# Totoro97/f2-nerf

Measured on AMD Instinct MI355X. Metric: training ray-samples/s (ngp_fox), higher is better.
Workload: dtype f16; 1 GPU; ngp_fox wanjinyou.yaml, 8192 rays/batch/GPU, 2^19 x16 table, the first 2188 iterations of training from the fresh-initialised table (fineness 8.7), synthetic random-pose rays, full train step (fwd+bwd+Adam+octree update); rays_per_batch=8192, parallelism=ray-dp1

## Files before the change

f2-nerf_amd/capi.py:

```python
import ctypes
import os

import torch

from . import build

_lib = None
ABI_VERSION = 13


class F2nError(RuntimeError):
    pass


def lib():
    global _lib
    if _lib is None:
        if not os.path.exists(build.LIB):
            raise F2nError("native library %s is missing: run `python -c 'import __graft_entry__ as g; g.build()'` "
                           "(there is no CPU fallback)" % build.LIB)
        _lib = ctypes.CDLL(build.LIB)
        _lib.f2n_build_info.restype = ctypes.c_char_p
        if _lib.f2n_abi_version() != ABI_VERSION:
            raise F2nError("%s reports ABI version %d, this binding is written for %d: rebuild (__graft_entry__.build())"
# ... 534 lines not shown

def flex_acc_bwd(n_rays, include_this, dsum, se, out):
    _ck(lib().f2n_flex_acc_bwd(_stream(), _i(n_rays), _i(int(include_this)), _p(dsum, "f32"), _p(se, "i32"), _p(out, "f32")),
        "f2n_flex_acc_bwd")


def adam_coefficients(step, lr, beta1=0.9, beta2=0.99, eps=1e-15, weight_decay=0.0, grad_scale=1.0):
    out = (ctypes.c_float * 9)()
    _ck(lib().f2n_adam_coefficients(_i(step), _f(lr), _d(beta1), _d(beta2), _f(eps), _f(weight_decay), _f(grad_scale), out),
        "f2n_adam_coefficients")
    return [float(v) for v in out]


def adam_step(n, param, grad, grad_scale, grad_round_h16, exp_avg, exp_avg_sq, step, lr, beta1, beta2, eps, wd, param_h,
              skip_flag=None, zero_grad=False):
    _ck(lib().f2n_adam_step(_stream(), _i(n), _p(param, "f32"), _p(grad, "f32"), _f(grad_scale), _i(int(grad_round_h16)),
                            _p(exp_avg, "f32"), _p(exp_avg_sq, "f32"), _i(step), _f(lr), _d(beta1), _d(beta2), _f(eps),
                            _f(wd), _p(param_h, "h16", True), _i(int(zero_grad)), _p(skip_flag, "i32", True)), "f2n_adam_step")


class _AdamGroup(ctypes.Structure):
    _fields_ = [("param", ctypes.c_void_p), ("grad", ctypes.c_void_p), ("exp_avg", ctypes.c_void_p), ("exp_avg_sq", ctypes.c_void_p),
                ("param_h", ctypes.c_void_p), ("n", ctypes.c_int), ("grad_scale", ctypes.c_float), ("weight_decay", ctypes.c_float),
                ("grad_round_h16", ctypes.c_int), ("check_finite", ctypes.c_int)]


def adam_small_groups(groups, step, lr, beta1, beta2, eps, zero_grad, flags=None, skip_flag=None):
    arr = (_AdamGroup * len(groups))()
    for a, g in zip(arr, groups):
        a.param = _p(g["param"], "f32").value
        a.grad = _p(g["grad"], "f32").value
        a.exp_avg = _p(g["exp_avg"], "f32").value
        a.exp_avg_sq = _p(g["exp_avg_sq"], "f32").value
        a.param_h = _p(g.get("param_h"), "h16", True).value
        a.n = int(g["param"].numel())
        a.grad_scale = float(g["grad_scale"])
        a.weight_decay = float(g["weight_decay"])
        a.grad_round_h16 = int(bool(g.get("grad_round_h16", False)))
        a.check_finite = int(bool(g.get("check_finite", False)))
    _ck(lib().f2n_adam_small_groups(_stream(), _i(len(groups)), arr, _i(step), _f(lr), _d(beta1), _d(beta2), _f(eps),
                                    _i(int(zero_grad)), _p(flags, "i32", True), _p(skip_flag, "i32", True)), "f2n_adam_small_groups")


def adam_fused(groups, table, step, lr, beta1, beta2, eps, zero_grad, skip_flag=None):
    arr = (_AdamGroup * max(len(groups), 1))()
    for a, g in zip(arr, groups):
        a.param = _p(g["param"], "f32").value
        a.grad = _p(g["grad"], "f32").value
        a.exp_avg = _p(g["exp_avg"], "f32").value
        a.exp_avg_sq = _p(g["exp_avg_sq"], "f32").value
        a.param_h = _p(g.get("param_h"), "h16", True).value
        a.n = int(g["param"].numel())
        a.grad_scale = float(g["grad_scale"])
        a.weight_decay = float(g["weight_decay"])
        a.grad_round_h16 = int(bool(g.get("grad_round_h16", False)))
        a.check_finite = 0
    t = table or {}
    _ck(lib().f2n_adam_fused(_stream(), _i(len(groups)), arr, _i(int(t.get("n", 0))), _p(t.get("param"), "f32", True),
                             _p(t.get("grad_h"), "h16", True), _f(float(t.get("grad_scale", 1.0))), _p(t.get("exp_avg"), "f32", True),
                             _p(t.get("exp_avg_sq"), "f32", True), _p(t.get("param_h"), "h16", True), _i(step), _f(lr), _d(beta1),
                             _d(beta2), _f(eps), _i(int(zero_grad)), _p(skip_flag, "i32", True)), "f2n_adam_fused")


def field_bwd_dyn(n_max, n_dev, n_off, n_volumes, prim_pool, local_idx, local_size, bias_pool, level_scale, pts_warped, volume_idx,
                  vol_stride, mlp_params_h, saved_x_h, dfeat, loss_scale, dparams_scaled, grad_table_h, level_entries, defer_reduce):
    _ck(lib().f2n_field_bwd_dyn(_stream(), _i(n_max), _p(n_dev, "i32", True), _i(n_off), _i(n_volumes), _p(prim_pool, "i32"),
                                _p(local_idx, "i32"), _p(local_size, "i32"), _p(bias_pool, "f32"), _p(level_scale, "f32"),
                                _p(pts_warped, "f32"), _p(volume_idx, "i32"), _i(vol_stride), _p(mlp_params_h, "h16"),
                                _p(saved_x_h, "h16"), _p(dfeat, "f32"), _f(loss_scale), _p(dparams_scaled, "f32"),
                                _p(grad_table_h, "h16"), _i(level_entries), _i(int(defer_reduce))), "f2n_field_bwd_dyn")


def field_bwd_dyn_rows(n_max, n_dev, n_off, n_volumes, prim_pool, local_idx, local_size, bias_pool, level_scale, pts_warped, volume_idx,
                       vol_stride, mlp_params_h, x_edge_h, x_cache_h, src_rows, dfeat, loss_scale, dparams_scaled, grad_table_h,
                       level_entries, defer_reduce):
    _ck(lib().f2n_field_bwd_dyn_rows(_stream(), _i(n_max), _p(n_dev, "i32", True), _i(n_off), _i(n_volumes), _p(prim_pool, "i32"),
                                     _p(local_idx, "i32"), _p(local_size, "i32"), _p(bias_pool, "f32"), _p(level_scale, "f32"),
                                     _p(pts_warped, "f32"), _p(volume_idx, "i32"), _i(vol_stride), _p(mlp_params_h, "h16"),
                                     _p(x_edge_h, "h16", True), _p(x_cache_h, "h16"), _p(src_rows, "i32"), _p(dfeat, "f32"),
                                     _f(loss_scale), _p(dparams_scaled, "f32"), _p(grad_table_h, "h16"), _i(level_entries),
                                     _i(int(defer_reduce))), "f2n_field_bwd_dyn_rows")


class _StepTail(ctypes.Structure):
    _fields_ = [("n_flags_a", ctypes.c_int), ("flags_grad_a", ctypes.c_void_p), ("n_flags_b", ctypes.c_int), ("flags_grad_b", ctypes.c_void_p),
                ("flags", ctypes.c_void_p), ("flags_mirror", ctypes.c_void_p), ("n_groups", ctypes.c_int), ("groups", ctypes.c_void_p),
                ("n_table", ctypes.c_int), ("table_param", ctypes.c_void_p), ("table_exp_avg", ctypes.c_void_p),
                ("table_exp_avg_sq", ctypes.c_void_p), ("table_param_h", ctypes.c_void_p), ("table_grad_scale", ctypes.c_float),
                ("step", ctypes.c_int), ("lr", ctypes.c_float), ("beta1", ctypes.c_double), ("beta2", ctypes.c_double), ("eps", ctypes.c_float),
                ("after_reduce", ctypes.c_void_p), ("after_reduce_user", ctypes.c_void_p), ("leave_table_to_caller", ctypes.c_int)]


def field_bwd_step_tail(n_max, n_dev, n_off, n_volumes, prim_pool, local_idx, local_size, bias_pool, level_scale, pts_warped, volume_idx,
                        vol_stride, mlp_params_h, saved_x_h, dfeat, loss_scale, dparams_scaled, grad_table_h, level_entries, flags_a,
                        flags_b, flags, groups, table, step, lr, beta1, beta2, eps, tail_stream=None, flags_mirror=None, leave_table_to_caller=False,
                        after_reduce=None, x_cache_h=None, src_rows=None):
    arr = (_AdamGroup * max(len(groups), 1))()
    for a, g in zip(arr, groups):
        a.param = _p(g["param"], "f32").value
        a.grad = _p(g["grad"], "f32").value
        a.exp_avg = _p(g["exp_avg"], "f32").value
        a.exp_avg_sq = _p(g["exp_avg_sq"], "f32").value
        a.param_h = _p(g.get("param_h"), "h16", True).value
        a.n = int(g["param"].numel())
        a.grad_scale = float(g["grad_scale"])
        a.weight_decay = float(g["weight_decay"])
        a.grad_round_h16 = int(bool(g.get("grad_round_h16", False)))
        a.check_finite = 0
    t = _StepTail()
    t.n_flags_a, t.flags_grad_a = int(flags_a.numel()), _p(flags_a, "f32").value
    t.n_flags_b, t.flags_grad_b = int(flags_b.numel()), _p(flags_b, "f32").value
    t.flags, t.flags_mirror = _p(flags, "i32").value, _mapped(flags_mirror).value
    t.n_groups, t.groups = len(groups), ctypes.cast(arr, ctypes.c_void_p).value
    t.n_table = int(table["n"])
    t.table_param, t.table_exp_avg, t.table_exp_avg_sq = _p(table["param"], "f32").value, _p(table["exp_avg"], "f32").value, _p(table["exp_avg_sq"], "f32").value
    t.table_param_h, t.table_grad_scale = _p(table["param_h"], "h16").value, float(table["grad_scale"])
    t.step, t.lr, t.beta1, t.beta2, t.eps = int(step), float(lr), float(beta1), float(beta2), float(eps)
    t.leave_table_to_caller = int(bool(leave_table_to_caller))
    cb = None
    if after_reduce is not None:
        cb = ctypes.CFUNCTYPE(None, ctypes.c_void_p, ctypes.c_void_p)(lambda user, chain: after_reduce(chain))
        t.after_reduce = ctypes.cast(cb, ctypes.c_void_p).value
    by_owners = ctypes.c_int(0)
    ts = ctypes.c_void_p(tail_stream.cuda_stream) if tail_stream is not None else ctypes.c_void_p(0)
    if x_cache_h is not None:
        _ck(lib().f2n_field_bwd_step_tail_rows(_stream(), ts, _i(n_max), _p(n_dev, "i32", True), _i(n_off), _i(n_volumes), _p(prim_pool, "i32"),
                                               _p(local_idx, "i32"), _p(local_size, "i32"), _p(bias_pool, "f32"), _p(level_scale, "f32"),
                                               _p(pts_warped, "f32"), _p(volume_idx, "i32"), _i(vol_stride), _p(mlp_params_h, "h16"),
                                               _p(saved_x_h, "h16", True), _p(x_cache_h, "h16"), _p(src_rows, "i32"), _p(dfeat, "f32"),
                                               _f(loss_scale), _p(dparams_scaled, "f32"), _p(grad_table_h, "h16"), _i(level_entries),
                                               ctypes.byref(t), ctypes.byref(by_owners)), "f2n_field_bwd_step_tail_rows")
        return by_owners.value
    _ck(lib().f2n_field_bwd_step_tail(_stream(), ts, _i(n_max), _p(n_dev, "i32", True), _i(n_off), _i(n_volumes), _p(prim_pool, "i32"),
                                      _p(local_idx, "i32"), _p(local_size, "i32"), _p(bias_pool, "f32"), _p(level_scale, "f32"),
                                      _p(pts_warped, "f32"), _p(volume_idx, "i32"), _i(vol_stride), _p(mlp_params_h, "h16"),
                                      _p(saved_x_h, "h16"), _p(dfeat, "f32"), _f(loss_scale), _p(dparams_scaled, "f32"),
                                      _p(grad_table_h, "h16"), _i(level_entries), ctypes.byref(t), ctypes.byref(by_owners)),
        "f2n_field_bwd_step_tail")
    return by_owners.value


def reduce_deferred():
    _ck(lib().f2n_reduce_deferred(_stream()), "f2n_reduce_deferred")


def deferred_reset():
    _ck(lib().f2n_deferred_reset(), "f2n_deferred_reset")


def adam_step_h16grad(n, param, grad_h, grad_scale, exp_avg, exp_avg_sq, step, lr, beta1, beta2, eps, wd, param_h,
                      zero_grad, skip_flag=None):
    _ck(lib().f2n_adam_step_h16grad(_stream(), _i(n), _p(param, "f32"), _p(grad_h, "h16"), _f(grad_scale),
                                    _p(exp_avg, "f32"), _p(exp_avg_sq, "f32"), _i(step), _f(lr), _d(beta1), _d(beta2),
                                    _f(eps), _f(wd), _p(param_h, "h16"), _i(int(zero_grad)),
                                    _p(skip_flag, "i32", True)), "f2n_adam_step_h16grad")


def train_loss(n_rays, pred, gt, disparity, sampled_var, n_edge, feat_dim, edge_feats, var_w, disp_w, tv_w, out_losses,
               dcolors, ddisparity, dvar, dedge_feats):
    _ck(lib().f2n_train_loss(_stream(), _i(n_rays), _p(pred, "f32"), _p(gt, "f32"), _p(disparity, "f32", True),
                             _p(sampled_var, "f32", True), _i(n_edge), _i(feat_dim), _p(edge_feats, "f32", True), _f(var_w),
                             _f(disp_w), _f(tv_w), _p(out_losses, "f32"), _p(dcolors, "f32", True), _p(ddisparity, "f32", True),
                             _p(dvar, "f32", True), _p(dedge_feats, "f32", True)), "f2n_train_loss")


def composite_train(n_rays, se, f0, f0_stride, dt, t, rgb, bg, gt, var_w, disp_w, tv_w, gs_progress, n_edge, feat_dim, edge_feats,
                    dedge_feats, colors, weights, drgb, df0, df0_stride, out_losses, defer_reduce=False):
    _ck(lib().f2n_composite_train(_stream(), _i(n_rays), _p(se, "i32"), _p(f0, "f32"), _i(f0_stride), _p(dt, "f32"), _p(t, "f32"),
                                  _p(rgb, "f32"), _p(bg, "f32"), _p(gt, "f32"), _f(var_w), _f(disp_w), _f(tv_w), _f(gs_progress),
                                  _i(n_edge), _i(feat_dim), _p(edge_feats, "f32", True), _p(dedge_feats, "f32", True),
                                  _p(colors, "f32"), _p(weights, "f32"), _p(drgb, "f32"), _p(df0, "f32"), _i(df0_stride),
                                  _p(out_losses, "f32"), _i(1 if defer_reduce else 0)), "f2n_composite_train")


def nonfinite_flags(n_a, a, n_b, b, flags, mirror=None):
    _ck(lib().f2n_nonfinite_flags_ex(_stream(), _i(n_a), _p(a, "f32", True), _i(n_b), _p(b, "f32", True), _p(flags, "i32"),
                                     _mapped(mirror)), "f2n_nonfinite_flags_ex")


def _lo3(lo):
    return (_f * 3)(*(float(v) for v in lo))


def oct_locate_warp(n, pts_world, tree_nodes, transes, out_pts, out_anchors):
    _ck(lib().f2n_oct_locate_warp(_stream(), _i(n), _p(pts_world, "f32"), _p(tree_nodes, "u8"), _p(transes, "u8"), _p(out_pts, "f32"),
                                  _p(out_anchors, "i32")), "f2n_oct_locate_warp")


def oct_locate_warp_grid(lo, step, nx, ny, nz, first_z, n_z, tree_nodes, transes, out_pts, out_anchors):
    _ck(lib().f2n_oct_locate_warp_grid(_stream(), _lo3(lo), _f(step), _i(nx), _i(ny), _i(nz), _i(first_z), _i(n_z), _p(tree_nodes, "u8"),
                                       _p(transes, "u8"), _p(out_pts, "f32"), _p(out_anchors, "i32")), "f2n_oct_locate_warp_grid")


def located_compact(n, anchors, pts_warped, counts, start_end, total, out_pts, out_vol, out_src=None):
    _ck(lib().f2n_located_compact(_stream(), _i(n), _p(anchors, "i32"), _p(pts_warped, "f32"), _p(counts, "i32"), _p(start_end, "i32"),
                                  _p(total, "i32"), _p(out_pts, "f32"), _p(out_vol, "i32"), _p(out_src, "i32", True)),
        "f2n_located_compact")


def density_scatter(n, anchors, start_end, f0, density):
    _ck(lib().f2n_density_scatter(_stream(), _i(n), _p(anchors, "i32"), _p(start_end, "i32"), _p(f0, "f32"), _p(density, "f32")),
        "f2n_density_scatter")


def field_density_grad(n, n_volumes, table_h, prim_pool, local_idx, local_size, bias_pool, level_scale, pts_warped, volume_idx, vol_stride,
                       mlp_params_h, x_h, out_dx, out_df0_dw):
    _ck(lib().f2n_field_density_grad(_stream(), _i(n), _i(n_volumes), _p(table_h, "h16"), _p(prim_pool, "i32"), _p(local_idx, "i32"),
# ... 550 lines not shown
```

f2-nerf_amd/csrc/field.hip:

```cpp
#include <math.h>
#include <atomic>
#include <string.h>

#include "adam_dev.h"
#include "mlp_dev.h"

struct F2nHashArgs {
  const half_t* table;
  const int32_t* prim_pool;
  const float* bias_pool;
  int n_volumes;
};

struct F2nLevelTab {
  float scale[F2N_N_LEVELS];
  int32_t base[F2N_N_LEVELS];
  uint32_t size[F2N_N_LEVELS];
};

__device__ __forceinline__ void f2n_level_tab_fill(F2nLevelTab& s, const float* level_scale, const int32_t* local_idx,
                                                   const int32_t* local_size, int tid) {
  if (tid < F2N_N_LEVELS) {
    s.scale[tid] = level_scale[tid];
    s.base[tid] = local_idx[tid];
// ... 959 lines not shown
  return f2n_rowfrag(x, F2N_D_IN, s, 0, g);
}
__device__ __forceinline__ half8_t f2n_load_xfrag_f32(const float* __restrict__ x, int s, int g, bool valid) {
  half8_t r = {0, 0, 0, 0, 0, 0, 0, 0};
  if (valid) {
    const float4_t lo = *(const float4_t*) (x + (size_t) s * F2N_D_IN + 4 * g);
    const float4_t hi = *(const float4_t*) (x + (size_t) s * F2N_D_IN + 16 + 4 * g);
#pragma unroll
    for (int i = 0; i < 4; i++) {
      r[i] = (half_t) lo[i];
      r[4 + i] = (half_t) hi[i];
    }
  }
  return r;
}
__device__ __forceinline__ void f2n_store_xfrag_h(half_t* __restrict__ x, int s, int g, half8_t xf) {
  half_t* p = x + (size_t) s * F2N_D_IN + 4 * g;
  *(half4_t*) p = __builtin_shufflevector(xf, xf, 0, 1, 2, 3);
  *(half4_t*) (p + 16) = __builtin_shufflevector(xf, xf, 4, 5, 6, 7);
}

#define F2N_FWD_THREADS 256

template <int NH, bool DO_HASH, bool DO_MLP>
__global__ __launch_bounds__(F2N_FWD_THREADS) void field_fwd_kernel(
    int n, F2nHashArgs h, const int32_t* __restrict__ local_idx, const int32_t* __restrict__ local_size,
    const float* __restrict__ level_scale, const float* __restrict__ pts, int pts_are_warped,
    const int32_t* __restrict__ volume_idx, int vol_stride, const float* __restrict__ x_f32,
    const half_t* __restrict__ params, float* __restrict__ out_feat_f32, half_t* __restrict__ out_feat_h,
    float* __restrict__ out_f0, half_t* __restrict__ save_x, const half_t* __restrict__ x_planes,
    const half_t* __restrict__ x_cache, const int32_t* __restrict__ src_rows, const int32_t* __restrict__ n_dev) {
  F2N_RAISE_PRIO();
  __shared__ F2nLevelTab lt;
  const int tid = threadIdx.x, lane = tid & 63, c = lane & 15, g = lane >> 4;
  const int n_alloc = n;
  if (n_dev != nullptr) n = min(n, *n_dev);
  if (DO_HASH) {
    f2n_level_tab_fill(lt, level_scale, local_idx, local_size, tid);
    __syncthreads();
  }
  F2nMlpFwdW<NH> w;
  if (DO_MLP) w.load(params, c, g);
  const int n_blocks = (n + 15) / 16;
  const int wave_global = blockIdx.x * (F2N_FWD_THREADS / 64) + (tid >> 6);
  const int wave_stride = gridDim.x * (F2N_FWD_THREADS / 64);
  for (int blk = wave_global; blk < n_blocks; blk += wave_stride) {
    const int s = blk * 16 + c;
    const bool valid = s < n;
    const int sc = valid ? s : n - 1;
    half8_t xf;
    if (DO_HASH) {
      float p01[3];
      f2n_load_point(pts, sc, pts_are_warped != 0, p01);
      const int vol = volume_idx[(size_t) sc * vol_stride];
      xf = f2n_gather_frag(h, lt, p01, vol, g, valid);
    } else if (x_planes != nullptr) {
      xf = f2n_cat(*(const half4_t*) (x_planes + ((size_t) g * n_alloc + sc) * 4),
                   *(const half4_t*) (x_planes + ((size_t) (4 + g) * n_alloc + sc) * 4));
      if (!valid) xf = half8_t{0, 0, 0, 0, 0, 0, 0, 0};
    } else if (x_cache != nullptr) {
      xf = f2n_load_xfrag_h(x_cache, src_rows != nullptr ? src_rows[sc] : sc, g, valid);
    } else {
      xf = f2n_load_xfrag_f32(x_f32, sc, g, valid);
    }
    if (save_x != nullptr && valid) f2n_store_xfrag_h(save_x, s, g, xf);
    if (DO_MLP) {
      const float4_t o = w.forward(xf);
      if (valid) {
        half4_t oh;
        float4_t of;
#pragma unroll
        for (int r = 0; r < 4; r++) {
          oh[r] = (half_t) o[r];
          of[r] = (float) oh[r];
        }
        if (out_feat_f32 != nullptr) *(float4_t*) (out_feat_f32 + (size_t) s * F2N_D_OUT + 4 * g) = of;
        if (out_feat_h != nullptr) *(half4_t*) (out_feat_h + (size_t) s * F2N_D_OUT + 4 * g) = oh;
        if (out_f0 != nullptr && g == 0) out_f0[s] = of[0];
      }
    }
  }
}

#define F2N_BWD_THREADS 256

template <int NH>
union F2nBwdSmem {
  F2nMlpLds<NH> w;
  float acc[2 * (F2N_D_HID * F2N_D_IN + (NH == 2 ? F2N_D_HID * F2N_D_HID : 0) + F2N_D_OUT * F2N_D_HID)];
};

template <int NH, int HASH, bool ROWS>
__device__ __forceinline__ void f2n_field_bwd_body(
    int n, F2nHashArgs h, const int32_t* __restrict__ local_idx, const int32_t* __restrict__ local_size,
    const float* __restrict__ level_scale, const float* __restrict__ pts, int pts_are_warped,
    const int32_t* __restrict__ volume_idx, int vol_stride, const half_t* __restrict__ params,
    const half_t* __restrict__ x_h, const float* __restrict__ x_f32, const float* __restrict__ dy, float loss_scale,
    float* __restrict__ dparams, float* __restrict__ dx_f32, half_t* __restrict__ grad_table, half_t* __restrict__ dx_planes,
    uint16_t* __restrict__ nz_mask, const int32_t* __restrict__ n_dev, int n_off, const half_t* __restrict__ x_cache,
    const int32_t* __restrict__ src_rows) {
  F2N_RAISE_PRIO();
  const int n_alloc = n;
  if (n_dev != nullptr) n = min(n, *n_dev + n_off);
  __shared__ F2nBwdSmem<NH> sm;
  __shared__ F2nLevelTab lt;
  const int tid = threadIdx.x, lane = tid & 63, c = lane & 15, g = lane >> 4;
  if (HASH == 1) f2n_level_tab_fill(lt, level_scale, local_idx, local_size, tid);
  f2n_mlp_lds_fill<NH>(sm.w, params, tid, F2N_BWD_THREADS);
  __syncthreads();
  const half8_t idf[2] = {f2n_identity_frag(0, c, g), f2n_identity_frag(1, c, g)};
  F2nMlpGradAcc<NH> acc;
  acc.zero();
  const int wave_global = blockIdx.x * (F2N_BWD_THREADS / 64) + (tid >> 6);
  const int wave_stride = gridDim.x * (F2N_BWD_THREADS / 64);
  const float inv_scale = 1.f / loss_scale;
  struct In {
    half8_t xf;
    float4_t d4;
  };
  auto fetch_row = [&](int tile) {
    const int s = tile * 16 + c;
    const int sc = s < n ? s : n - 1;
    return sc < n_off ? -1 : src_rows[sc - n_off];
  };
  auto fetch = [&](int tile, int row, In& o) {
    const int s = tile * 16 + c;
    const int sc = s < n ? s : n - 1;
    if (ROWS) o.xf = f2n_rowfrag(row >= 0 ? x_cache + (size_t) row * F2N_D_IN : x_h + (size_t) sc * F2N_D_IN, F2N_D_IN, 0, 0, g);
    else o.xf = (x_h != nullptr) ? f2n_load_xfrag_h(x_h, sc, g, true) : f2n_load_xfrag_f32(x_f32, sc, g, true);
    o.d4 = *(const float4_t*) (dy + (size_t) sc * F2N_D_OUT + 4 * g);
  };
  const int n_tiles = (n + 15) / 16;
  In cur;
  int row_next = 0;
  if (wave_global < n_tiles) {
    if (ROWS) row_next = fetch_row(wave_global);
    fetch(wave_global, row_next, cur);
    if (ROWS) row_next = fetch_row(wave_global + wave_stride < n_tiles ? wave_global + wave_stride : wave_global);
  }
  for (int tile = wave_global; tile < n_tiles; tile += wave_stride) {
    In nxt;
    const int t1 = tile + wave_stride < n_tiles ? tile + wave_stride : tile;
    fetch(t1, row_next, nxt);
    if (ROWS) row_next = fetch_row(t1 + wave_stride < n_tiles ? t1 + wave_stride : t1);
    __builtin_amdgcn_sched_barrier(0);
    {
      F2nHalfBwd<NH> hb;
      int lds_off = 0;
      asm volatile("" : "+v"(lds_off));
      const F2nMlpLds<NH>& wl = *(const F2nMlpLds<NH>*) ((const char*) &sm.w + lds_off);
      const int s = tile * 16 + c;
      const bool valid = s < n;
      const int sc = valid ? s : n - 1;
      const half8_t xf = valid ? cur.xf : half8_t{0, 0, 0, 0, 0, 0, 0, 0};
      half8_t dyf = {0, 0, 0, 0, 0, 0, 0, 0};
#pragma unroll
      for (int r = 0; r < 4; r++)
        dyf[r] = valid ? (half_t) ((float) (half_t) cur.d4[r] * loss_scale) : (half_t) 0.f;
      f2n_mlp_half_bwd<NH, 2>(wl, xf, [&](half8_t, half8_t) { return dyf; }, idf, c, g, hb);
      if (valid) {
        if (dx_f32 != nullptr) {
#pragma unroll
          for (int ft = 0; ft < 2; ft++) {
            float4_t v;
#pragma unroll
            for (int r = 0; r < 4; r++) v[r] = hb.dxT[ft][r] * inv_scale;
            *(float4_t*) (dx_f32 + (size_t) s * F2N_D_IN + 16 * ft + 4 * g) = v;
          }
        }
      }
      if (HASH != 0) {
        half8_t gx = f2n_pack<false>(hb.dxT[0], hb.dxT[1]);
        if (HASH == 2) {
          bool nz = false;
#pragma unroll
          for (int e = 0; e < 8; e++) nz |= (float) gx[e] != 0.f;
          const unsigned long long bal = __ballot(nz && valid);
          if (valid) {
            *(half4_t*) (dx_planes + ((size_t) g * n_alloc + s) * 4) = __builtin_shufflevector(gx, gx, 0, 1, 2, 3);
            *(half4_t*) (dx_planes + ((size_t) (4 + g) * n_alloc + s) * 4) = __builtin_shufflevector(gx, gx, 4, 5, 6, 7);
          }
          if (lane == 0)
            nz_mask[tile] = (uint16_t) ((bal | (bal >> 16) | (bal >> 32) | (bal >> 48)) & 0xffffull);
        } else {
          float p01[3];
          f2n_load_point(pts, sc, pts_are_warped != 0, p01);
          const int vol = volume_idx[(size_t) sc * vol_stride];
          if (!valid) gx = half8_t{0, 0, 0, 0, 0, 0, 0, 0};
          f2n_scatter_frag(h, lt, grad_table, p01, vol, g, c, gx);
        }
      }
      f2n_mlp_accumulate_dw_half<NH>(hb, acc);
    }
    cur = nxt;
  }
  __syncthreads();
  f2n_mlp_flush_dw<NH>(acc, sm.acc, dparams, c, g, tid, F2N_BWD_THREADS);
}

template <int NH, int HASH, int BPC>
__global__ __launch_bounds__(F2N_BWD_THREADS, BPC) void field_bwd_kernel(
    int n, F2nHashArgs h, const int32_t* __restrict__ local_idx, const int32_t* __restrict__ local_size,
    const float* __restrict__ level_scale, const float* __restrict__ pts, int pts_are_warped,
    const int32_t* __restrict__ volume_idx, int vol_stride, const half_t* __restrict__ params,
    const half_t* __restrict__ x_h, const float* __restrict__ x_f32, const float* __restrict__ dy, float loss_scale,
    float* __restrict__ dparams, float* __restrict__ dx_f32, half_t* __restrict__ grad_table, half_t* __restrict__ dx_planes,
    uint16_t* __restrict__ nz_mask, const int32_t* __restrict__ n_dev, int n_off) {
  f2n_field_bwd_body<NH, HASH, false>(n, h, local_idx, local_size, level_scale, pts, pts_are_warped, volume_idx, vol_stride, params, x_h,
                                      x_f32, dy, loss_scale, dparams, dx_f32, grad_table, dx_planes, nz_mask, n_dev, n_off, nullptr,
                                      nullptr);
}

template <int HASH, int BPC>
__global__ __launch_bounds__(F2N_BWD_THREADS, BPC) void field_bwd_rows_kernel(
    int n, F2nHashArgs h, const int32_t* __restrict__ local_idx, const int32_t* __restrict__ local_size,
    const float* __restrict__ level_scale, const float* __restrict__ pts, int pts_are_warped,
    const int32_t* __restrict__ volume_idx, int vol_stride, const half_t* __restrict__ params,
    const half_t* __restrict__ x_edge, const half_t* __restrict__ x_cache, const int32_t* __restrict__ src_rows,
    const float* __restrict__ dy, float loss_scale, float* __restrict__ dparams, half_t* __restrict__ grad_table,
    half_t* __restrict__ dx_planes, uint16_t* __restrict__ nz_mask, const int32_t* __restrict__ n_dev, int n_off) {
  f2n_field_bwd_body<1, HASH, true>(n, h, local_idx, local_size, level_scale, pts, pts_are_warped, volume_idx, vol_stride, params, x_edge,
                                    nullptr, dy, loss_scale, dparams, nullptr, grad_table, dx_planes, nz_mask, n_dev, n_off, x_cache,
                                    src_rows);
}

__global__ __launch_bounds__(256) void hash_bwd_kernel(int n, F2nHashArgs h, const int32_t* __restrict__ local_idx,
                                                       const int32_t* __restrict__ local_size,
                                                       const float* __restrict__ level_scale, const float* __restrict__ pts,
                                                       int pts_are_warped, const int32_t* __restrict__ volume_idx,
                                                       int vol_stride, const half_t* __restrict__ grad_in,
                                                       half_t* __restrict__ grad_table) {
  __shared__ F2nLevelTab lt;
  const int tid = threadIdx.x, lane = tid & 63, c = lane & 15, g = lane >> 4;
  f2n_level_tab_fill(lt, level_scale, local_idx, local_size, tid);
  __syncthreads();
  const int n_blocks = (n + 15) / 16;
  const int wave_global = blockIdx.x * 4 + (tid >> 6);
  const int wave_stride = gridDim.x * 4;
  for (int blk = wave_global; blk < n_blocks; blk += wave_stride) {
    const int s = blk * 16 + c;
    const bool valid = s < n;
    const int sc = valid ? s : n - 1;
    float p01[3];
    f2n_load_point(pts, sc, pts_are_warped != 0, p01);
    const int vol = volume_idx[(size_t) sc * vol_stride];
    half8_t gx = f2n_rowfrag(grad_in, F2N_D_IN, sc, 0, g);
    if (!valid) gx = half8_t{0, 0, 0, 0, 0, 0, 0, 0};
    f2n_scatter_frag(h, lt, grad_table, p01, vol, g, c, gx);
  }
}

__global__ void mlp_init_kernel(uint64_t seed, int d_in, int d_hidden, int n_hidden, float* __restrict__ params) {
  const int i = blockIdx.x * blockDim.x + threadIdx.x;
  const int n0 = d_hidden * d_in, n1 = (n_hidden - 1) * d_hidden * d_hidden, no = F2N_D_OUT * d_hidden;
  if (i >= n0 + n1 + no) return;
  int fan_in, fan_out;
  if (i < n0) { fan_in = d_in; fan_out = d_hidden; }
  else if (i < n0 + n1) { fan_in = d_hidden; fan_out = d_hidden; }
  else { fan_in = d_hidden; fan_out = F2N_D_OUT; }
  uint64_t zz = seed + 0x9e3779b97f4a7c15ull * (uint64_t) (i + 1);
  zz = (zz ^ (zz >> 30)) * 0xbf58476d1ce4e5b9ull;
  zz = (zz ^ (zz >> 27)) * 0x94d049bb133111ebull;
  zz = zz ^ (zz >> 31);
  const float u = (float) (zz >> 40) * (1.f / 16777216.f);
  const float scale = sqrtf(6.f / (float) (fan_in + fan_out));
  params[i] = (u * 2.f - 1.f) * scale;
}

__global__ void to_h16_kernel(int n, const float* __restrict__ in, half_t* __restrict__ out) {
  const int i = blockIdx.x * blockDim.x + threadIdx.x;
  if (i < n) out[i] = (half_t) in[i];
}

__global__ __launch_bounds__(256) void mlp_input_grad_kernel(int n, const half_t* __restrict__ params, const half_t* __restrict__ x_h,
                                                             float* __restrict__ dx_rows, float* __restrict__ dx_planes) {
  __shared__ float s_w1[F2N_D_HID * F2N_D_IN];
  __shared__ float s_g[F2N_D_HID];
  const int tid = threadIdx.x;
  for (int i = tid; i < F2N_D_HID * F2N_D_IN; i += 256) s_w1[i] = (float) params[i];
  if (tid < F2N_D_HID) s_g[tid] = (float) params[F2N_D_HID * F2N_D_IN + tid];
  __syncthreads();
  for (int64_t s = (int64_t) blockIdx.x * 256 + tid; s < n; s += (int64_t) gridDim.x * 256) {
    float x[F2N_D_IN], dx[F2N_D_IN];
#pragma unroll
    for (int v = 0; v < 4; v++) {
      const half8_t xv = *(const half8_t*) (x_h + s * F2N_D_IN + 8 * v);
#pragma unroll
      for (int i = 0; i < 8; i++) x[8 * v + i] = (float) xv[i];
    }
#pragma unroll
    for (int k = 0; k < F2N_D_IN; k++) dx[k] = 0.f;
#pragma unroll 2
    for (int j = 0; j < F2N_D_HID; j++) {
      const float* w = s_w1 + F2N_D_IN * j;
      float pre = w[0] * x[0];
#pragma unroll
      for (int k = 1; k < F2N_D_IN; k++) pre = pre + w[k] * x[k];
      const float gj = pre > 0.f ? s_g[j] : 0.f;
#pragma unroll
      for (int k = 0; k < F2N_D_IN; k++) dx[k] = dx[k] + w[k] * gj;
    }
    if (dx_rows != nullptr) {
#pragma unroll
      for (int p = 0; p < 8; p++)
        *(float4_t*) (dx_rows + s * F2N_D_IN + 4 * p) = float4_t{dx[4 * p], dx[4 * p + 1], dx[4 * p + 2], dx[4 * p + 3]};
    }
// ... 469 lines not shown
  if (n == 0) return F2N_OK;
  F2nHashArgs h = {(const half_t*) table_h, prim_pool, bias_pool, n_volumes};
  long per_part = ((long) n + 255) / 256;
  if (per_part > 256) per_part = 256;
  const size_t stage_bytes = (size_t) 2 * n_volumes * 6 * sizeof(uint32_t);
  F2nGatherPlan plan;
  float cost8[F2N_N_PARTS];
  const int variant = f2n_gather_variant(n, n_volumes, step01, level_scale_host, cost8);
  const bool staged = (variant & 1) != 0, balanced = (variant & 2) != 0;
  f2n_gather_plan((n + 255) / 256, balanced ? cost8 : nullptr, plan);
#define F2N_LAUNCH_GATHER(ST, CB)                                                                                              \
  hipLaunchKernelGGL((hash_gather_planes_kernel<ST, CB>), dim3((unsigned) (F2N_N_PARTS * per_part)), dim3(256),                \
                     ST ? stage_bytes : 0, (hipStream_t) stream, n, h, local_idx, local_size, level_scale, pts, pts_are_warped, \
                     volume_idx, vol_stride, (half_t*) planes_h, plan)
  if (staged && balanced) F2N_LAUNCH_GATHER(true, true);
  else if (staged) F2N_LAUNCH_GATHER(true, false);
  else if (balanced) F2N_LAUNCH_GATHER(false, true);
  else F2N_LAUNCH_GATHER(false, false);
#undef F2N_LAUNCH_GATHER
  return f2n_launch_status();
}

int f2n_hash_gather_planes_binned(void* stream, int n, int n_volumes, const void* table_h, const int32_t* prim_pool,
                                  const int32_t* local_idx, const int32_t* local_size, const float* bias_pool,
                                  const float* level_scale, const float* pts, int pts_are_warped, const int32_t* volume_idx,
                                  int vol_stride, void* planes_h, int level_entries, int first_binned_pair) {
  const int p0 = first_binned_pair;
  if (n < 0 || n_volumes <= 0 || vol_stride < 1 || p0 < 0 || p0 > F2N_N_PARTS) return F2N_ERR_INVALID_ARG;
  if (level_entries < F2N_N_PARTS * F2N_GB_ENTRIES || (level_entries & (level_entries - 1)) != 0 || (level_entries >> F2N_GB_SHIFT) > F2N_GB_MAX_BINS)
    return F2N_ERR_UNSUPPORTED;
  if (n == 0) return F2N_OK;
  hipStream_t st = (hipStream_t) stream;
  F2nHashArgs h = {(const half_t*) table_h, prim_pool, bias_pool, n_volumes};
  const int n_tiles = (n + 255) / 256;
  if (p0 > 0) {
    long per_part = n_tiles;
    if (per_part > 256) per_part = 256;
    F2nGatherPlan plan;
    f2n_gather_plan_coarse(n_tiles, p0, plan);
    hipLaunchKernelGGL((hash_gather_planes_kernel<false, false>), dim3((unsigned) (F2N_N_PARTS * per_part)), dim3(256), 0, st, n, h,
                       local_idx, local_size, level_scale, pts, pts_are_warped, volume_idx, vol_stride, (half_t*) planes_h, plan);
    const int rc = f2n_launch_status();
    if (rc != F2N_OK) return rc;
  }
  if (p0 == F2N_N_PARTS) return F2N_OK;
  F2nGatherBins q;
  q.l0 = 2 * p0;
  const int nl = F2N_N_LEVELS - q.l0;
  q.n_bins = level_entries >> F2N_GB_SHIFT;
  q.nc = (n + F2N_GB_CHUNK - 1) / F2N_GB_CHUNK;
  if (q.nc > F2N_GB_MAX_CHUNKS) return F2N_ERR_UNSUPPORTED;
  const size_t n_regions = (size_t) nl * q.nc;
  auto up = [](size_t b) { return (b + 255) & ~(size_t) 255; };
  const size_t b_res = up(n_regions * F2N_GB_REGION * sizeof(uint32_t)), b_req = up(n_regions * F2N_GB_REGION * sizeof(uint16_t));
  const size_t b_offc = up(n_regions * q.n_bins * sizeof(uint16_t));
  const size_t b_total = up(n_regions * sizeof(int32_t)), b_slots = up((size_t) nl * n * 8 * sizeof(uint16_t));
  char* ws = (char*) f2n_ws_get(F2N_WS_GATHER_BINS, b_res + b_req + b_offc + b_total + b_slots);
  if (ws == nullptr) return F2N_ERR_INVALID_ARG;
  q.res = (uint32_t*) ws;
  q.req = (uint16_t*) (ws + b_res);
  q.offc = (uint16_t*) (ws + b_res + b_req);
  q.total = (int32_t*) (ws + b_res + b_req + b_offc);
  q.slots = (uint16_t*) (ws + b_res + b_req + b_offc + b_total);
  hipLaunchKernelGGL(gather_request_kernel, dim3(nl * q.nc), dim3(F2N_GB_THREADS), 0, st, n, h, local_idx, local_size, level_scale,
                     pts, pts_are_warped, volume_idx, vol_stride, q);
  if (F2N_GB_REGION / q.n_bins > 40)
    hipLaunchKernelGGL((gather_serve_kernel<16, 4>), dim3(nl * q.n_bins), dim3(F2N_GB_SERVE_THREADS), 0, st, (const half_t*) table_h, local_idx, q);
  else
    hipLaunchKernelGGL((gather_serve_kernel<8, 4>), dim3(nl * q.n_bins), dim3(F2N_GB_SERVE_THREADS), 0, st, (const half_t*) table_h, local_idx, q);
  hipLaunchKernelGGL(gather_blend_kernel, dim3((F2N_N_PARTS - p0) * q.nc), dim3(F2N_GB_THREADS), 0, st, n, h, local_idx, local_size,
                     level_scale, pts, pts_are_warped, volume_idx, vol_stride, (half_t*) planes_h, q);
  return f2n_launch_status();
}

int f2n_field_mlp_planes(void* stream, int n, const void* planes_h, const void* mlp_params_h, float* out_feat_f32, float* out_f0,
                         void* save_x_h) {
  return f2n_field_mlp_planes_ex(stream, n, planes_h, mlp_params_h, out_feat_f32, out_f0, save_x_h, nullptr);
}

int f2n_field_mlp_planes_ex(void* stream, int n, const void* planes_h, const void* mlp_params_h, float* out_feat_f32, float* out_f0,
                            void* save_x_h, void* out_feat_h) {
  if (n < 0 || (n > 0 && planes_h == nullptr)) return F2N_ERR_INVALID_ARG;
  if (n == 0) return F2N_OK;
  F2nHashArgs h = {nullptr, nullptr, nullptr, 1};
  hipLaunchKernelGGL((field_fwd_kernel<1, false, true>), dim3(f2n_wave_grid((n + 15) / 16, 4)), dim3(F2N_FWD_THREADS), 0,
                     (hipStream_t) stream, n, h, nullptr, nullptr, nullptr, nullptr, 0, nullptr, 1, nullptr,
                     (const half_t*) mlp_params_h, out_feat_f32, (half_t*) out_feat_h, out_f0, (half_t*) save_x_h, (const half_t*) planes_h,
                     nullptr, nullptr, nullptr);
  return f2n_launch_status();
}

int f2n_hash_pos_grad(void* stream, int n, int n_volumes, const void* table_h, const int32_t* prim_pool, const int32_t* local_idx,
                      const int32_t* local_size, const float* bias_pool, const float* level_scale, const float* pts_warped,
                      const int32_t* volume_idx, int vol_stride, const float* dx, float* out_df0_dw) {
  if (n < 0 || n_volumes <= 0 || vol_stride < 1) return F2N_ERR_INVALID_ARG;
  if (n == 0) return F2N_OK;
  if (dx == nullptr || out_df0_dw == nullptr || ((uintptr_t) dx & 15)) return F2N_ERR_INVALID_ARG;
  F2nHashArgs h = {(const half_t*) table_h, prim_pool, bias_pool, n_volumes};
  return f2n_pos_grad_launch((hipStream_t) stream, n, h, local_idx, local_size, level_scale, pts_warped, volume_idx, vol_stride, dx,
                             F2N_D_IN, 4, out_df0_dw);
}

int f2n_field_density_grad(void* stream, int n, int n_volumes, const void* table_h, const int32_t* prim_pool, const int32_t* local_idx,
                           const int32_t* local_size, const float* bias_pool, const float* level_scale, const float* pts_warped,
                           const int32_t* volume_idx, int vol_stride, const void* mlp_params_h, const void* x_h, float* out_dx,
                           float* out_df0_dw) {
  if (n < 0 || n_volumes <= 0 || vol_stride < 1) return F2N_ERR_INVALID_ARG;
  if (n == 0) return F2N_OK;
  if (mlp_params_h == nullptr || x_h == nullptr || out_df0_dw == nullptr || ((uintptr_t) x_h & 15) || ((uintptr_t) out_dx & 15))
    return F2N_ERR_INVALID_ARG;
  float* planes = (float*) f2n_ws_get(F2N_WS_DGRAD_DX, sizeof(float) * F2N_D_IN * (size_t) n);
  if (planes == nullptr) return F2N_ERR_INVALID_ARG;
  long blocks = ((long) n + 255) / 256;
  if (blocks > 2048) blocks = 2048;
  hipLaunchKernelGGL(mlp_input_grad_kernel, dim3((unsigned) blocks), dim3(256), 0, (hipStream_t) stream, n, (const half_t*) mlp_params_h,
                     (const half_t*) x_h, out_dx, planes);
  const int rc = f2n_launch_status();
  if (rc != F2N_OK) return rc;
  F2nHashArgs h = {(const half_t*) table_h, prim_pool, bias_pool, n_volumes};
  return f2n_pos_grad_launch((hipStream_t) stream, n, h, local_idx, local_size, level_scale, pts_warped, volume_idx, vol_stride, planes,
                             4, 4 * (size_t) n, out_df0_dw);
}

int f2n_field_fwd_cached(void* stream, int n, int n_cache, const int32_t* src_rows, const void* x_cache_h,
                         const void* mlp_params_h, float* out_feat_f32, float* out_f0, void* save_x_h) {
  return f2n_field_fwd_cached_dyn(stream, n, nullptr, n_cache, src_rows, x_cache_h, mlp_params_h, out_feat_f32, out_f0, save_x_h);
}

int f2n_field_fwd_cached_dyn(void* stream, int n_max, const int32_t* n_dev, int n_cache, const int32_t* src_rows,
                             const void* x_cache_h, const void* mlp_params_h, float* out_feat_f32, float* out_f0, void* save_x_h) {
  const int n = n_max;
  if (n < 0 || n_cache < 0 || (n > 0 && x_cache_h == nullptr) || (src_rows == nullptr && n > n_cache)) return F2N_ERR_INVALID_ARG;
  if (n == 0) return F2N_OK;
  F2nHashArgs h = {nullptr, nullptr, nullptr, 1};
  hipLaunchKernelGGL((field_fwd_kernel<1, false, true>), dim3(f2n_wave_grid((n + 15) / 16, 4)), dim3(F2N_FWD_THREADS), 0,
                     (hipStream_t) stream, n, h, nullptr, nullptr, nullptr, nullptr, 0, nullptr, 1, nullptr,
                     (const half_t*) mlp_params_h, out_feat_f32, nullptr, out_f0, (half_t*) save_x_h, nullptr,
                     (const half_t*) x_cache_h, src_rows, n_dev);
  return f2n_launch_status();
}

int f2n_field_bwd(void* stream, int n, int n_volumes, const int32_t* prim_pool, const int32_t* local_idx,
                  const int32_t* local_size, const float* bias_pool, const float* level_scale, const float* pts_warped,
                  const int32_t* volume_idx, int vol_stride, const void* mlp_params_h, const void* saved_x_h,
                  const float* dfeat, float loss_scale, float* dparams_f32_scaled, void* grad_table_h, int level_entries) {
  return f2n_field_bwd_dyn(stream, n, nullptr, 0, n_volumes, prim_pool, local_idx, local_size, bias_pool, level_scale, pts_warped,
                           volume_idx, vol_stride, mlp_params_h, saved_x_h, dfeat, loss_scale, dparams_f32_scaled, grad_table_h,
                           level_entries, 0);
}

static int f2n_field_bwd_impl(void* stream, void* tail_stream, int n_max, const int32_t* n_dev, int n_off, int n_volumes,
                              const int32_t* prim_pool, const int32_t* local_idx, const int32_t* local_size, const float* bias_pool,
                              const float* level_scale, const float* pts_warped, const int32_t* volume_idx, int vol_stride,
                              const void* mlp_params_h, const void* saved_x_h, const float* dfeat, float loss_scale,
                              float* dparams_f32_scaled, void* grad_table_h, int level_entries, int defer_reduce,
                              const F2nStepTail* tail, int* table_stepped, const void* x_cache_h = nullptr,
                              const int32_t* src_rows = nullptr) {
  const int n = n_max;
  if (table_stepped != nullptr) *table_stepped = 0;
  if (n < 0 || n_volumes <= 0 || vol_stride < 1 || !(loss_scale > 0.f) || level_entries < 0 || ((uintptr_t) mlp_params_h & 15))
    return F2N_ERR_INVALID_ARG;
  if (x_cache_h != nullptr && (src_rows == nullptr || n_off < 0 || n_off > n || (n_off > 0 && saved_x_h == nullptr))) return F2N_ERR_INVALID_ARG;
  if (tail != nullptr && (tail->flags == nullptr || tail->n_groups < 0 || tail->n_groups > 4 || tail->step < 1 || tail->n_table < 0 ||
                          (tail->n_table > 0 && (tail->table_param == nullptr || tail->table_exp_avg == nullptr ||
                                                 tail->table_exp_avg_sq == nullptr || tail->table_param_h == nullptr))))
    return F2N_ERR_INVALID_ARG;
  if (n == 0 && tail == nullptr) return F2N_OK;
  F2nHashArgs h = {nullptr, prim_pool, bias_pool, n_volumes};
  const bool bins = n > 0 && f2n_use_bins(n, level_entries);
  int rc = F2N_OK;
  const int n_params = f2n_mlp_n_params(F2N_D_IN, F2N_D_HID, 1);
  half_t* dx_planes = nullptr;
  uint16_t* nz_mask = nullptr;
  if (n > 0) {
    const unsigned blocks = f2n_bwd_grid((n + 31) / 32, bins ? 3 : 2);
    float* partials = (float*) f2n_ws_get(F2N_WS_FIELD_DW, sizeof(float) * (size_t) blocks * n_params);
    if (partials == nullptr) return F2N_ERR_INVALID_ARG;
    if (bins) {
      const size_t plane_bytes = sizeof(half_t) * 32 * (size_t) n;
      dx_planes = (half_t*) f2n_ws_get(F2N_WS_FIELD_PLANES, plane_bytes + sizeof(uint16_t) * ((size_t) n / 16 + 2));
      if (dx_planes == nullptr) return F2N_ERR_INVALID_ARG;
      nz_mask = (uint16_t*) ((char*) dx_planes + plane_bytes);
    }
#define F2N_LAUNCH_FIELD_BWD(HASH, BPC)                                                                                      \
  hipLaunchKernelGGL((field_bwd_kernel<1, HASH, BPC>), dim3(blocks), dim3(F2N_BWD_THREADS), 0, (hipStream_t) stream, n, h,  \
                     local_idx, local_size, level_scale, pts_warped, 1, volume_idx, vol_stride, (const half_t*) mlp_params_h, \
                     (const half_t*) saved_x_h, nullptr, dfeat, loss_scale, partials, nullptr, (half_t*) grad_table_h,       \
                     dx_planes, nz_mask, n_dev, n_off)
#define F2N_LAUNCH_FIELD_BWD_ROWS(HASH, BPC)                                                                                   \
  hipLaunchKernelGGL((field_bwd_rows_kernel<HASH, BPC>), dim3(blocks), dim3(F2N_BWD_THREADS), 0, (hipStream_t) stream, n, h,   \
                     local_idx, local_size, level_scale, pts_warped, 1, volume_idx, vol_stride, (const half_t*) mlp_params_h,  \
                     (const half_t*) saved_x_h, (const half_t*) x_cache_h, src_rows, dfeat, loss_scale, partials,             \
                     (half_t*) grad_table_h, dx_planes, nz_mask, n_dev, n_off)
    if (x_cache_h != nullptr) {
      if (!bins) F2N_LAUNCH_FIELD_BWD_ROWS(1, 2);
      else F2N_LAUNCH_FIELD_BWD_ROWS(2, 3);
    } else if (!bins) F2N_LAUNCH_FIELD_BWD(1, 2);
    else F2N_LAUNCH_FIELD_BWD(2, 3);
#undef F2N_LAUNCH_FIELD_BWD
#undef F2N_LAUNCH_FIELD_BWD_ROWS
    rc = f2n_launch_status();
    if (rc != F2N_OK) return rc;
    if (tail == nullptr && !defer_reduce) {
      if (dx_planes != nullptr) {
        rc = f2n_binned_scatter((hipStream_t) stream, n, h, local_idx, local_size, level_scale, pts_warped, 1, volume_idx, vol_stride,
                                dx_planes, 4, 4 * (long) n, nz_mask, (half_t*) grad_table_h, level_entries, n_dev, n_off);
        if (rc != F2N_OK) return rc;
      }
      return f2n_reduce_partials(stream, n_params, (int) blocks, partials, dparams_f32_scaled);
    }
    rc = f2n_defer_reduction(n_params, (int) blocks, partials, dparams_f32_scaled);
    if (rc != F2N_OK) return rc;
  }
  if (tail == nullptr) {
    if (dx_planes == nullptr) return F2N_OK;
    return f2n_binned_scatter((hipStream_t) stream, n, h, local_idx, local_size, level_scale, pts_warped, 1, volume_idx, vol_stride, dx_planes,
                              4, 4 * (long) n, nz_mask, (half_t*) grad_table_h, level_entries, n_dev, n_off);
  }
  hipStream_t st = (hipStream_t) stream, ts = tail_stream != nullptr ? (hipStream_t) tail_stream : st;
  hipEvent_t ev_fork = nullptr, ev_join = nullptr;
  if (ts != st) {
    int dev = 0;
    static hipEvent_t evs[16][2];
    static bool made[16];
    if (hipGetDevice(&dev) != hipSuccess || dev < 0 || dev >= 16) return F2N_ERR_INVALID_ARG;
    if (!made[dev]) {
      if (hipEventCreateWithFlags(&evs[dev][0], hipEventDisableTiming) != hipSuccess || hipEventCreateWithFlags(&evs[dev][1], hipEventDisableTiming) != hipSuccess)
        return F2N_ERR_UNSUPPORTED;
      made[dev] = true;
    }
    ev_fork = evs[dev][0];
    ev_join = evs[dev][1];
    if (hipEventRecord(ev_fork, st) != hipSuccess || hipStreamWaitEvent(ts, ev_fork, 0) != hipSuccess) return F2N_ERR_INVALID_ARG;
  }
  rc = f2n_reduce_deferred(ts);
  if (rc != F2N_OK) return rc;
  if (tail->after_reduce != nullptr) tail->after_reduce(tail->after_reduce_user, (void*) ts);
  rc = f2n_nonfinite_flags_ex(ts, tail->n_flags_a, tail->flags_grad_a, tail->n_flags_b, tail->flags_grad_b, tail->flags, tail->flags_mirror);
  if (rc != F2N_OK) return rc;
  const int32_t* skip = tail->flags + 2;
  rc = f2n_adam_fused(ts, tail->n_groups, tail->groups, 0, nullptr, nullptr, 1.f, nullptr, nullptr, nullptr, tail->step, tail->lr, tail->beta1,
                      tail->beta2, tail->eps, 1, skip);
  if (rc != F2N_OK) return rc;
  if (ts != st && hipEventRecord(ev_join, ts) != hipSuccess) return F2N_ERR_INVALID_ARG;
  int by_owners = 0;
  if (dx_planes != nullptr) {
    const long S = (long) (F2N_N_LEVELS + 1) * ((level_entries >> F2N_BIN_SHIFT) / 2);
    F2nOwnerAdam ad;
    ad.param = (float2*) tail->table_param;
    ad.exp_avg = (float2*) tail->table_exp_avg;
    ad.exp_avg_sq = (float2*) tail->table_exp_avg_sq;
    ad.param_h = (half2_t*) tail->table_param_h;
    ad.k = f2n_adam_coef(tail->step, tail->lr, tail->beta1, tail->beta2, tail->eps, 0.f, tail->table_grad_scale);
    ad.skip = skip;
    const bool can = !tail->leave_table_to_caller && tail->n_table > 0 && (long) tail->n_table == S * 2 * F2N_BIN_ENTRIES;
    rc = f2n_binned_scatter(st, n, h, local_idx, local_size, level_scale, pts_warped, 1, volume_idx, vol_stride, dx_planes, 4, 4 * (long) n, nz_mask,
                            (half_t*) grad_table_h, level_entries, n_dev, n_off, can ? &ad : nullptr, ev_join, &by_owners);
    if (rc != F2N_OK) return rc;
  }
  if (!by_owners) {
    if (ts != st && hipStreamWaitEvent(st, ev_join, 0) != hipSuccess) return F2N_ERR_INVALID_ARG;
    if (tail->n_table > 0 && !tail->leave_table_to_caller) {
      rc = f2n_adam_fused(st, 0, nullptr, tail->n_table, tail->table_param, grad_table_h, tail->table_grad_scale, tail->table_exp_avg,
                          tail->table_exp_avg_sq, tail->table_param_h, tail->step, tail->lr, tail->beta1, tail->beta2, tail->eps, 1, skip);
      if (rc != F2N_OK) return rc;
    }
  }
  if (table_stepped != nullptr) *table_stepped = by_owners;
  return F2N_OK;
}

int f2n_field_bwd_dyn(void* stream, int n_max, const int32_t* n_dev, int n_off, int n_volumes, const int32_t* prim_pool,
                      const int32_t* local_idx, const int32_t* local_size, const float* bias_pool, const float* level_scale,
                      const float* pts_warped, const int32_t* volume_idx, int vol_stride, const void* mlp_params_h,
                      const void* saved_x_h, const float* dfeat, float loss_scale, float* dparams_f32_scaled, void* grad_table_h,
                      int level_entries, int defer_reduce) {
  return f2n_field_bwd_impl(stream, nullptr, n_max, n_dev, n_off, n_volumes, prim_pool, local_idx, local_size, bias_pool, level_scale, pts_warped,
                            volume_idx, vol_stride, mlp_params_h, saved_x_h, dfeat, loss_scale, dparams_f32_scaled, grad_table_h, level_entries,
                            defer_reduce, nullptr, nullptr);
}

int f2n_field_bwd_step_tail(void* stream, void* tail_stream, int n_max, const int32_t* n_dev, int n_off, int n_volumes,
                            const int32_t* prim_pool, const int32_t* local_idx, const int32_t* local_size, const float* bias_pool,
                            const float* level_scale, const float* pts_warped, const int32_t* volume_idx, int vol_stride,
                            const void* mlp_params_h, const void* saved_x_h, const float* dfeat, float loss_scale,
                            float* dparams_f32_scaled, void* grad_table_h, int level_entries, const F2nStepTail* tail,
                            int* table_stepped_by_owners) {
  if (tail == nullptr) return F2N_ERR_INVALID_ARG;
  return f2n_field_bwd_impl(stream, tail_stream, n_max, n_dev, n_off, n_volumes, prim_pool, local_idx, local_size, bias_pool, level_scale,
                            pts_warped, volume_idx, vol_stride, mlp_params_h, saved_x_h, dfeat, loss_scale, dparams_f32_scaled, grad_table_h,
                            level_entries, 1, tail, table_stepped_by_owners);
}

int f2n_field_bwd_dyn_rows(void* stream, int n_max, const int32_t* n_dev, int n_off, int n_volumes, const int32_t* prim_pool,
                           const int32_t* local_idx, const int32_t* local_size, const float* bias_pool, const float* level_scale,
                           const float* pts_warped, const int32_t* volume_idx, int vol_stride, const void* mlp_params_h,
                           const void* x_edge_h, const void* x_cache_h, const int32_t* src_rows, const float* dfeat, float loss_scale,
                           float* dparams_f32_scaled, void* grad_table_h, int level_entries, int defer_reduce) {
  if (x_cache_h == nullptr) return F2N_ERR_INVALID_ARG;
  return f2n_field_bwd_impl(stream, nullptr, n_max, n_dev, n_off, n_volumes, prim_pool, local_idx, local_size, bias_pool, level_scale, pts_warped,
                            volume_idx, vol_stride, mlp_params_h, x_edge_h, dfeat, loss_scale, dparams_f32_scaled, grad_table_h, level_entries,
                            defer_reduce, nullptr, nullptr, x_cache_h, src_rows);
}

int f2n_field_bwd_step_tail_rows(void* stream, void* tail_stream, int n_max, const int32_t* n_dev, int n_off, int n_volumes,
                                 const int32_t* prim_pool, const int32_t* local_idx, const int32_t* local_size, const float* bias_pool,
                                 const float* level_scale, const float* pts_warped, const int32_t* volume_idx, int vol_stride,
                                 const void* mlp_params_h, const void* x_edge_h, const void* x_cache_h, const int32_t* src_rows,
                                 const float* dfeat, float loss_scale, float* dparams_f32_scaled, void* grad_table_h, int level_entries,
                                 const F2nStepTail* tail, int* table_stepped_by_owners) {
  if (tail == nullptr || x_cache_h == nullptr) return F2N_ERR_INVALID_ARG;
  return f2n_field_bwd_impl(stream, tail_stream, n_max, n_dev, n_off, n_volumes, prim_pool, local_idx, local_size, bias_pool, level_scale,
                            pts_warped, volume_idx, vol_stride, mlp_params_h, x_edge_h, dfeat, loss_scale, dparams_f32_scaled, grad_table_h,
                            level_entries, 1, tail, table_stepped_by_owners, x_cache_h, src_rows);
}

}
```

f2-nerf_amd/csrc/host/Field.cpp:

```cpp
#include "Hash3DAnchored.h"

#include <cstdlib>

namespace f2n {

using torch::autograd::AutogradContext;
using torch::autograd::variable_list;

FusedMLP::FusedMLP(GlobalDataPool* gdp, int d_in, int d_out, int d_hidden, int n_hidden_layers) {
  global_data_pool_ = gdp;
  d_in_ = d_in; d_out_ = d_out; d_hidden_ = d_hidden; n_hidden_layers_ = n_hidden_layers;
  n_params_ = f2n_mlp_n_params(d_in, d_hidden, n_hidden_layers);
  TORCH_CHECK(n_params_ > 0 && d_out <= F2N_MLP_OUT_PAD, "unsupported MLP shape");
  params_ = torch::zeros({n_params_}, DevF32());
  params_h_ = torch::zeros({n_params_}, DevF16());
  grad_scaled_ = torch::zeros({n_params_}, DevF32());
  InitParams();
  params_.requires_grad_(true);
}

void FusedMLP::InitParams() {
  torch::NoGradGuard g;
  const uint64_t seed = 19970826;
  F2N_CALL(f2n_mlp_init_params(CurStream(), seed + (uint64_t) n_hidden_layers_, d_in_, d_hidden_, n_hidden_layers_,
// ... 184 lines not shown
    auto* f = reinterpret_cast<Hash3DAnchored*>(ctx->saved_data["field"].toInt());
    auto saved = ctx->get_saved_variables();
    const int n = saved[0].size(0);
    Tensor gin = (grad_output[0] * 128.f).to(torch::kFloat16).contiguous();
    f->grad_clean_ = false;
    F2N_TIMED_CALL("hash_bwd", f2n_hash_bwd(CurStream(), n, f->n_volumes_, I32P(f->prim_pool_), I32P(f->feat_local_idx_), I32P(f->feat_local_size_),
                          F32P(f->bias_pool_), F32P(f->level_scale_), F32P(saved[0]), 1, I32P(saved[1]),
                          (int) ctx->saved_data["stride"].toInt(), VoidP(gin), VoidP(f->grad_h_), f->pool_size_ / N_LEVELS));
    return {Tensor(), Tensor(), Tensor(), Tensor()};
  }
};

}

Tensor Hash3DAnchored::HashEncode(const Tensor& points, const Tensor& anchors) {
  Tensor pts = points.contiguous();
  CheckDev(pts, torch::kFloat32, "points");
  return HashEncodeFunction::apply(feat_pool_, pts, anchors, reinterpret_cast<int64_t>(this))[0];
}

void Hash3DAnchored::DensityGrad(const Tensor& points, const Tensor& vol, const Tensor& x_h, Tensor& g) {
  F2N_TIMED_CALL("field_density_grad", f2n_field_density_grad(CurStream(), (int) points.size(0), n_volumes_, VoidP(feat_pool_h_), I32P(prim_pool_),
                         I32P(feat_local_idx_), I32P(feat_local_size_), F32P(bias_pool_), F32P(level_scale_), F32P(points), I32P(vol), 1,
                         VoidP(mlp_->params_h_), VoidP(x_h), nullptr, F32P(g)));
}

void Hash3DAnchored::PosGrad(const Tensor& points, const Tensor& vol, const Tensor& dx, Tensor& g) {
  F2N_CALL(f2n_hash_pos_grad(CurStream(), (int) points.size(0), n_volumes_, VoidP(feat_pool_h_), I32P(prim_pool_), I32P(feat_local_idx_),
                             I32P(feat_local_size_), F32P(bias_pool_), F32P(level_scale_), F32P(points), I32P(vol), 1, F32P(dx), F32P(g)));
}

void Hash3DAnchored::ForwardRaw(const Tensor& points, const Tensor& anchors, int stride, const Tensor& src_rows, int n_reuse,
                                Tensor& feat, Tensor& saved_x, Tensor* f0_cached) {
  const int n = points.size(0);
  const int n_cached = n_reuse, n_tail = n - n_cached;
  if (n_cached > 0) {
    TORCH_CHECK(prepass_x_.defined() && src_rows.numel() >= n_cached, "no pre-pass feature cache for this query");
    F2N_TIMED_CALL("field_fwd_cached", f2n_field_fwd_cached(CurStream(), n_cached, (int) prepass_x_.size(0), I32P(src_rows),
                           VoidP(prepass_x_), VoidP(mlp_->params_h_), F32P(feat), f0_cached != nullptr ? F32P(*f0_cached) : nullptr,
                           VoidP(saved_x)));
  }
  if (n_tail > 0)
    F2N_TIMED_CALL("field_fwd", f2n_field_fwd(CurStream(), n_tail, n_volumes_, VoidP(feat_pool_h_), I32P(prim_pool_),
                           I32P(feat_local_idx_), I32P(feat_local_size_), F32P(bias_pool_), F32P(level_scale_),
                           F32P(points) + 3 * (int64_t) n_cached, I32P(anchors) + (int64_t) stride * n_cached, stride,
                           VoidP(mlp_->params_h_), F32P(feat) + (int64_t) F2N_MLP_OUT_PAD * n_cached, nullptr,
                           static_cast<void*>(saved_x.data_ptr<at::Half>() + (int64_t) N_LEVELS * N_CHANNELS * n_cached)));
}

void Hash3DAnchored::BackwardRaw(const Tensor& points, const Tensor& anchors, int stride, const Tensor& saved_x, const Tensor& dfeat) {
  const int n = points.size(0);
  grad_clean_ = false;
  F2N_TIMED_CALL("field_bwd", f2n_field_bwd(CurStream(), n, n_volumes_, I32P(prim_pool_), I32P(feat_local_idx_),
                         I32P(feat_local_size_), F32P(bias_pool_), F32P(level_scale_), F32P(points), I32P(anchors), stride,
                         VoidP(mlp_->params_h_), VoidP(saved_x), F32P(dfeat), mlp_->loss_scale_, F32P(mlp_->grad_scaled_),
                         VoidP(grad_h_), pool_size_ / N_LEVELS));
}

Tensor Hash3DAnchored::AnchoredQuery(const Tensor& points, const Tensor& anchors) {
  Tensor pts = points.contiguous();
  CheckDev(pts, torch::kFloat32, "points");
  if (!fused_ok_) return mlp_->Query(HashEncode(pts, anchors));
  Tensor feat = FieldFunction::apply(feat_pool_, mlp_->params_, pts, anchors, torch::empty({0}, DevI32()), (int64_t) 0,
                                     reinterpret_cast<int64_t>(this))[0];
  return mlp_out_dim_ == F2N_MLP_OUT_PAD ? feat : feat.index({Slc(), Slc(0, mlp_out_dim_)}).contiguous();
}

Tensor Hash3DAnchored::AnchoredQueryReuse(const Tensor& points, const Tensor& anchors, const Tensor& src_rows, int n_reuse) {
  Tensor pts = points.contiguous();
  CheckDev(pts, torch::kFloat32, "points");
  Tensor rows = src_rows.contiguous();
  CheckDev(rows, torch::kInt32, "src_rows");
  TORCH_CHECK(n_reuse >= 0 && n_reuse <= pts.size(0) && rows.numel() >= n_reuse, "bad reuse range");
  if (!fused_ok_) {
    DropPrepassCache();
    return AnchoredQuery(pts, anchors);
  }
  Tensor feat = FieldFunction::apply(feat_pool_, mlp_->params_, pts, anchors, rows.slice(0, 0, n_reuse), (int64_t) n_reuse,
                                     reinterpret_cast<int64_t>(this))[0];
  DropPrepassCache();
  return mlp_out_dim_ == F2N_MLP_OUT_PAD ? feat : feat.index({Slc(), Slc(0, mlp_out_dim_)}).contiguous();
}

Tensor Hash3DAnchored::QueryDensityPreAct(const Tensor& points, const Tensor& anchors, bool keep_features, bool keep_outputs) {
  torch::NoGradGuard g;
  Tensor pts = points.contiguous();
  CheckDev(pts, torch::kFloat32, "points");
  AnchorView av = ViewAnchors(anchors);
  const int n = pts.size(0);
  if (!fused_ok_) {
    DropPrepassCache();
    return mlp_->Query(HashEncode(pts, anchors)).select(1, 0).contiguous();
  }
  Tensor f0 = torch::empty({n}, DevF32());
  prepass_x_ = keep_features ? torch::empty({n, N_LEVELS * N_CHANNELS}, DevF16()) : Tensor();
  prepass_feat_h_ = keep_features && keep_outputs ? torch::empty({n, F2N_MLP_OUT_PAD}, DevF16()) : Tensor();
  void* feat_h = prepass_feat_h_.defined() ? VoidP(prepass_feat_h_) : nullptr;
#if F2N_DEBUG_BUILD
  static const bool force_fused = []() {
    const char* e = std::getenv("F2N_FUSED_GATHER");
    return e != nullptr && e[0] == '1';
  }();
#else
  constexpr bool force_fused = false;
#endif
  if (force_fused) {
    F2N_TIMED_CALL("field_prepass_fused", f2n_field_fwd_fused_ex(CurStream(), n, n_volumes_, VoidP(feat_pool_h_), I32P(prim_pool_),
                           I32P(feat_local_idx_), I32P(feat_local_size_), F32P(bias_pool_), F32P(level_scale_), F32P(pts), I32P(av.t),
                           av.stride, VoidP(mlp_->params_h_), nullptr, F32P(f0), keep_features ? VoidP(prepass_x_) : nullptr, feat_h));
  } else if (n >= 32768) {
    Tensor planes = torch::empty({8, n, 4}, DevF16());
    const float step01 = march_step_warped_ * global_data_pool_->ray_march_fineness_ * .5f;
#if F2N_DEBUG_BUILD
    static const int binned_p0 = []() {
      const char* e = std::getenv("F2N_BINNED_GATHER_P0");
      const int v = e != nullptr ? std::atoi(e) : 1;
      return v < 0 ? 0 : (v > 8 ? 8 : v);
    }();
    static const int binned_min_log2 = []() {
      const char* e = std::getenv("F2N_BINNED_GATHER_MIN_LOG2");
      return e != nullptr ? std::atoi(e) : 20;
    }();
#else
    constexpr int binned_p0 = 1, binned_min_log2 = 20;
#endif
    const int level_entries = (int) (pool_size_ / N_LEVELS);
    if (binned_p0 < 8 && level_entries >= (1 << binned_min_log2) && level_entries <= (1 << 22) && n >= 65536 && n <= 1536 * 1024) {
      F2N_TIMED_CALL("hash_gather", f2n_hash_gather_planes_binned(CurStream(), n, n_volumes_, VoidP(feat_pool_h_), I32P(prim_pool_),
                             I32P(feat_local_idx_), I32P(feat_local_size_), F32P(bias_pool_), F32P(level_scale_), F32P(pts), 1,
                             I32P(av.t), av.stride, VoidP(planes), level_entries, binned_p0));
    } else {
      F2N_TIMED_CALL("hash_gather", f2n_hash_gather_planes_balanced(CurStream(), n, n_volumes_, VoidP(feat_pool_h_), I32P(prim_pool_),
                             I32P(feat_local_idx_), I32P(feat_local_size_), F32P(bias_pool_), F32P(level_scale_), F32P(pts), 1,
                             I32P(av.t), av.stride, VoidP(planes), balance_gather_ ? step01 : 0.f, level_scale_host_.data()));
    }
    F2N_TIMED_CALL("field_mlp_prepass", f2n_field_mlp_planes_ex(CurStream(), n, VoidP(planes), VoidP(mlp_->params_h_), nullptr, F32P(f0),
                           keep_features ? VoidP(prepass_x_) : nullptr, feat_h));
  } else {
    F2N_TIMED_CALL("field_prepass", f2n_field_fwd_ex(CurStream(), n, n_volumes_, VoidP(feat_pool_h_), I32P(prim_pool_), I32P(feat_local_idx_),
                           I32P(feat_local_size_), F32P(bias_pool_), F32P(level_scale_), F32P(pts), I32P(av.t), av.stride,
                           VoidP(mlp_->params_h_), nullptr, F32P(f0), keep_features ? VoidP(prepass_x_) : nullptr, feat_h));
  }
  return f0;
}

int Hash3DAnchored::LoadStates(const std::vector<Tensor>& states, int idx) {
  torch::NoGradGuard g;
  feat_pool_.copy_(states[idx++].to(torch::kCUDA).to(torch::kFloat32).reshape({pool_size_, N_CHANNELS}));
  prim_pool_ = states[idx++].clone().to(torch::kCUDA).to(torch::kInt32).contiguous();
  bias_pool_ = states[idx++].clone().to(torch::kCUDA).to(torch::kFloat32).contiguous();
  n_volumes_ = states[idx++].item<int>();
  TORCH_CHECK(prim_pool_.numel() == int64_t(N_LEVELS) * n_volumes_ * 3 && bias_pool_.numel() == int64_t(N_LEVELS) * n_volumes_ * 3,
              "prime/bias pools do not match n_volumes");
  mlp_->params_.copy_(states[idx++].to(torch::kCUDA).to(torch::kFloat32));
  SyncHalf();
  return idx;
}

std::vector<Tensor> Hash3DAnchored::States() {
  return {feat_pool_.detach(), prim_pool_, bias_pool_, torch::full({1}, n_volumes_, CpuI32()), mlp_->params_.detach()};
}

std::vector<ParamGroup> Hash3DAnchored::OptimParamGroups() {
  ParamGroup table;
  table.name = "feat_pool";
  table.param = feat_pool_;
  table.grad = grad_h_;
  table.param_h = feat_pool_h_;
  table.grad_scale = 1.f / 128.f;
  table.grad_is_h16 = true;
  table.active = active_halves_;
  ParamGroup mlp;
  mlp.name = "field_mlp";
  mlp.param = mlp_->params_;
  mlp.grad = mlp_->grad_scaled_;
  mlp.param_h = mlp_->params_h_;
  mlp.weight_decay = 1e-6f;
  mlp.grad_round_h16 = true;
  mlp.grad_scale = -1.f;
  return {table, mlp};
}

void Hash3DAnchored::Reset() {
  torch::NoGradGuard g;
  feat_pool_.uniform_(-1e-2f, 1e-2f);
  mlp_->InitParams();
  SyncHalf();
}

std::unique_ptr<Field> ConstructField(GlobalDataPool* gdp) {
  const std::string type = gdp->config_.Str("field.type");
  TORCH_CHECK(type == "Hash3DAnchored", "unknown field.type: ", type);
  return std::make_unique<Hash3DAnchored>(gdp);
}

}
```

f2-nerf_amd/csrc/host/Hash3DAnchored.h:

```cpp
#pragma once
#include "FusedMLP.h"

namespace f2n {

#define N_CHANNELS 2
#define N_LEVELS 16
#define RES_FINE_POW_2 10.f
#define RES_BASE_POW_2 3.f

class Hash3DAnchored : public Field {
 public:
  explicit Hash3DAnchored(GlobalDataPool* global_data_pool);
  Tensor AnchoredQuery(const Tensor& points, const Tensor& anchors) override;
  Tensor QueryDensityPreAct(const Tensor& points, const Tensor& anchors, bool keep_features = false, bool keep_outputs = false);
  void DropPrepassCache() { prepass_x_ = Tensor(); prepass_feat_h_ = Tensor(); }
  Tensor AnchoredQueryReuse(const Tensor& points, const Tensor& anchors, const Tensor& src_rows, int n_reuse);
  void ForwardRaw(const Tensor& points, const Tensor& anchors, int stride, const Tensor& src_rows, int n_reuse, Tensor& feat,
                  Tensor& saved_x, Tensor* f0_cached = nullptr);
  void BackwardRaw(const Tensor& points, const Tensor& anchors, int stride, const Tensor& saved_x, const Tensor& dfeat);

  int LoadStates(const std::vector<Tensor>& states, int idx) override;
  std::vector<Tensor> States() override;
  std::vector<ParamGroup> OptimParamGroups() override;
  void Reset() override;
  void SyncHalf();
  void ZeroGrad();
  bool fused_ok_ = true;
  Tensor HashEncode(const Tensor& points, const Tensor& anchors);
  void DensityGrad(const Tensor& points, const Tensor& vol, const Tensor& x_h, Tensor& g);
  void PosGrad(const Tensor& points, const Tensor& vol, const Tensor& dx, Tensor& g);
  Tensor TableGradUnscaled();

  int pool_size_;
  int mlp_hidden_dim_, mlp_out_dim_, n_hidden_layers_;
  Tensor feat_pool_;
  Tensor feat_pool_h_;
  Tensor grad_h_;
  Tensor prim_pool_;
  Tensor bias_pool_;
  Tensor feat_local_idx_, feat_local_size_, level_scale_;
  bool grad_clean_ = false;
  Tensor prepass_x_;
  Tensor prepass_feat_h_;
  std::unique_ptr<FusedMLP> mlp_;
  int n_volumes_;
  std::vector<float> level_scale_host_;
  float march_step_warped_ = 0.f;
  bool balance_gather_ = true;
  int64_t active_halves_;
};

}
```

f2-nerf_amd/csrc/host/Renderer.cpp:

```cpp
#include "Renderer.h"

#include <hip/hip_runtime_api.h>

#include <cstdio>
#include <cstdlib>
#include <mutex>

namespace f2n {

using torch::autograd::AutogradContext;
using torch::autograd::variable_list;

namespace {

struct CompositeFunction : public torch::autograd::Function<CompositeFunction> {
  static variable_list forward(AutogradContext* ctx, Tensor feat, Tensor rgb, Tensor dt, Tensor t, Tensor bg, Tensor se,
                               double gs_progress) {
    ctx->set_materialize_grads(false);
    const int n_rays = se.size(0), m = feat.size(0);
    Tensor colors = torch::empty({n_rays, 3}, DevF32()), disparity = torch::empty({n_rays}, DevF32());
    Tensor depth = torch::empty({n_rays}, DevF32()), weights = torch::empty({m}, DevF32());
    F2N_TIMED_CALL("composite_fwd", f2n_composite_fwd(CurStream(), n_rays, I32P(se), F32P(feat), F2N_MLP_OUT_PAD, F32P(dt), F32P(t), F32P(rgb), F32P(bg),
                               F32P(colors), F32P(disparity), F32P(depth), F32P(weights), nullptr));
    ctx->save_for_backward({feat, rgb, dt, t, bg, se});
// ... 221 lines not shown
  }
  spec_start_recorded_ = false;
  if (train) total_all_pts_ += n_all_pts;
  if (train) DigestBegin(n_rays, n_all_pts);
  if (train) gdp->sampled_pts_per_ray_ = gdp->sampled_pts_per_ray_ * 0.9f + (float(n_all_pts) / float(n_rays)) * 0.1f;

  RenderFront fr;
  fr.bg_color = bg_color;
  if (n_all_pts <= 0) {
    pack_done();
    const bool dp_lagged = train && dp_world_ > 1 && async_count;
    if (train && dp_world_ > 1 && !dp_lagged) dp_count_ = torch::zeros({1}, DevI32());
    if (train && static_cast<PersSampler*>(pts_sampler_.get())->occupancy_sync_hook_)
      pts_sampler_->UpdateOctNodes(sample_result_, torch::empty({0}, DevF32()), torch::empty({0}, DevF32()));
    if (dp_lagged) {
      Tensor total = torch::empty({1}, DevI32());
      n_kept_words_.Ensure(2);
      if (dp_count_.defined()) {
        F2N_CALL(f2n_segment_scan_ex(CurStream(), 0, nullptr, nullptr, I32P(total), n_kept_words_.Dev(0), I32P(dp_count_), 1));
        dp_sum_mirrored_ = true;
        dp_sum_rays_ = dp_count_rays_;
      } else {
        F2N_CALL(f2n_segment_scan_ex(CurStream(), 0, nullptr, nullptr, I32P(total), n_kept_words_.Dev(1), nullptr, 0));
      }
      kept_wait_ev_ = &n_kept_ev_;
      n_kept_ev_.record();
      dp_count_ = total;
      dp_count_rays_ = n_rays;
      count_pending_ = true;
      pending_count_rays_ = n_rays;
      pending_count_seq_ = cur_seq_;
    } else if (train && dp_world_ > 1) {
      if (!dp_count_host_.defined()) dp_count_host_ = torch::empty({1}, torch::TensorOptions().dtype(torch::kInt32).pinned_memory(true));
      dp_count_host_.copy_(dp_count_, true);
      dp_count_ev_.record();
    }
    if (train && !dp_lagged) {
      gdp->meaningful_sampled_pts_per_ray_ = gdp->meaningful_sampled_pts_per_ray_ * 0.9f + KeptPerRayForEma(0, n_rays) * 0.1f;
      RecordEma(cur_seq_);
      DigestKept(cur_seq_, 0);
    }
    last_n_kept_pts_ = 0;
    fr.empty = true;
    consumed_side_samples_ = false;
    octree_ready_ev_.record();
    return fr;
  }
  void* st = CurStream();

  SampleResultFlex& es = fr.es;
  Tensor &pts_all = fr.pts_all, &vol_all = fr.vol_all, &src_rows = fr.src_rows;
  int n_kept = 0;
  const int64_t front = 2 * (int64_t) n_edge;
  const bool edges_cached = async_count && n_edge > 0 && sample_result_.extra_rows >= front &&
                            sample_result_.pts.storage_offset() >= 3 * front && sample_result_.anchors.storage_offset() >= 3 * front;
  auto edge_samples_to = [&](float* pts1, int32_t* idx1, int stride1, float* pts2, int32_t* idx2) {
    auto& oct = *ps->pers_octree_;
    F2N_CALL(f2n_edge_samples_ex(st, n_edge, VoidP(oct.edge_pool_gpu_), oct.n_edges_, VoidP(oct.pers_trans_gpu_),
                                 edge_idx.defined() ? I32P(edge_idx) : nullptr, edge_coord.defined() ? F32P(edge_coord) : nullptr,
                                 edge_u.defined() ? F32P(edge_u) : nullptr, pts1, idx1, stride1, pts2, idx2, 1));
  };
  {
    torch::NoGradGuard no_grad;
    Tensor f0_full;
    const float* f0p = nullptr;
    if (edges_cached) {
      const int64_t n_rows = (int64_t) n_all_pts + front;
      Tensor pts_full = sample_result_.pts.as_strided({n_rows, 3}, {3, 1}, sample_result_.pts.storage_offset() - 3 * front);
      Tensor anchors_full = sample_result_.anchors.as_strided({n_rows, 3}, {3, 1}, sample_result_.anchors.storage_offset() - 3 * front);
      if (pregen) {
        pts_all = sample_result_.pts_all.narrow(0, 0, n_rows);
        vol_all = sample_result_.vol_all.narrow(0, 0, n_rows);
      } else {
        pts_all = torch::empty({n_rows, 3}, DevF32());
        vol_all = torch::empty({n_rows}, DevI32());
        edge_samples_to(F32P(pts_full), I32P(anchors_full), 3, F32P(pts_all), I32P(vol_all));
      }
      pack_done();
      if (digest_taps_ && train) {
        DigestTap(TAP_PTS_PRE, sample_result_.pts);
        DigestTap(TAP_DT_PRE, sample_result_.dt);
        DigestTap(TAP_ANCHORS_PRE, sample_result_.anchors.select(1, 0));
      }
      f0_full = field->QueryDensityPreAct(pts_full, anchors_full, true, keep_prepass_outputs_);
      f0p = F32P(f0_full) + front;
      if (digest_taps_ && train) DigestTap(TAP_EDGE, pts_full.narrow(0, 0, front));
      fr.edge_cache_row = 0;
      fr.sample_cache_row = front;
    } else {
      pack_done();
      if (digest_taps_ && train) {
        DigestTap(TAP_PTS_PRE, sample_result_.pts);
        DigestTap(TAP_DT_PRE, sample_result_.dt);
        DigestTap(TAP_ANCHORS_PRE, sample_result_.anchors.select(1, 0));
      }
      f0_full = field->QueryDensityPreAct(sample_result_.pts, sample_result_.anchors, true, keep_prepass_outputs_);
      f0p = F32P(f0_full);
    }
    if (digest_taps_ && train) {
      DigestTap(TAP_PTS, sample_result_.pts);
      DigestTap(TAP_DT, sample_result_.dt);
      DigestTap(TAP_ANCHORS, sample_result_.anchors.select(1, 0));
      DigestTap(TAP_F0, f0_full);
      DigestTap(TAP_BG, bg_color);
    }
    Tensor weights = torch::empty({n_all_pts}, DevF32()), alphas = torch::empty({n_all_pts}, DevF32());
    Tensor mask = torch::empty({n_all_pts}, DevI32()), kept = torch::empty({n_rays}, DevI32());
    if (train) ps->EarlyStopAndVote(sample_result_, f0p, weights, alphas, mask, kept);
    else F2N_TIMED_CALL("early_stop", f2n_early_stop(st, n_rays, I32P(sample_result_.pts_idx_bounds), f0p, 1, F32P(sample_result_.dt),
                            F32P(weights), F32P(alphas), I32P(mask), I32P(kept)));
    const bool octree_first = train && async_count;
    auto octree_update_issued = [&]() {
      octree_ready_ev_.record();
      const int nslot = next_batch_.valid ? FindPending(next_batch_.rays_o, next_batch_.rays_d) : -1;
      if (nslot >= 0 && pend_[nslot].s.speculative && !pend_[nslot].s.completed && PreSampleSpecComplete(nslot)) after_octree_update_ = nullptr;
      else if (nslot >= 0 && pend_[nslot].s.completed) after_octree_update_ = nullptr;
      if (after_octree_update_) {
        auto f = std::move(after_octree_update_);
        after_octree_update_ = nullptr;
        f();
      }
    };
    Tensor new_se = torch::empty({n_rays, 2}, DevI32()), total = torch::empty({1}, DevI32());
    n_kept_words_.Ensure(2);
    bool scan_issued = false;
    if (octree_first) {
      PersSampler::ScanArgs sa;
      sa.n = n_rays; sa.counts = I32P(kept); sa.start_end = I32P(new_se); sa.total = I32P(total);
      if (train && dp_world_ > 1 && dp_count_.defined()) {
        sa.mirror = n_kept_words_.Dev(0); sa.also = I32P(dp_count_); sa.n_also = 1;
        dp_sum_mirrored_ = true;
        dp_sum_rays_ = dp_count_rays_;
      } else {
        sa.mirror = n_kept_words_.Dev(1);
      }
      ps->FinishOctUpdate(&sa);
      scan_issued = true;
      octree_update_issued();
    }
    const bool dp_lagged = train && dp_world_ > 1 && octree_first;
    if (scan_issued) {
    } else if (dp_lagged && dp_count_.defined()) {
      F2N_CALL(f2n_segment_scan_ex(st, n_rays, I32P(kept), I32P(new_se), I32P(total), n_kept_words_.Dev(0), I32P(dp_count_), 1));
      dp_sum_mirrored_ = true;
      dp_sum_rays_ = dp_count_rays_;
    } else {
      F2N_CALL(f2n_segment_scan_ex(st, n_rays, I32P(kept), I32P(new_se), I32P(total), n_kept_words_.Dev(1), nullptr, 0));
    }
    kept_wait_ev_ = scan_issued ? &octree_ready_ev_ : &n_kept_ev_;
    if (!scan_issued) n_kept_ev_.record();
    if (digest_taps_ && train) DigestTap(TAP_SURVIVORS, new_se);
    if (dp_lagged) {
      dp_count_ = total;
      dp_count_rays_ = n_rays;
    } else if (train && dp_world_ > 1) {
      dp_count_ = total.clone();
    }
    if (train && !octree_first) ps->FinishOctUpdate();
    if (train && dp_world_ > 1 && !dp_lagged) {
      if (!dp_count_host_.defined()) dp_count_host_ = torch::empty({1}, torch::TensorOptions().dtype(torch::kInt32).pinned_memory(true));
      dp_count_host_.copy_(dp_count_, true);
      dp_count_ev_.record();
    }
    if (train && !octree_first) octree_update_issued();
    if (async_count) {
      n_kept = n_all_pts;
      if (train) {
        count_pending_ = true;
        pending_count_rays_ = n_rays;
        pending_count_seq_ = cur_seq_;
      }
      fr.dyn = true;
      fr.n_kept_dev = total;
    } else {
      kept_wait_ev_->synchronize();
      n_kept = n_kept_words_.Read(1);
      if (train && after_count_readback_) after_count_readback_();
      last_n_kept_pts_ = n_kept;
      if (train) total_kept_pts_ += n_kept;
// ... 144 lines not shown
```

f2-nerf_amd/csrc/host/Renderer.h:

```cpp
#pragma once
#include "Hash3DAnchored.h"
#include "PersSampler.h"

namespace f2n {

class SHShader : public Shader {
 public:
  explicit SHShader(GlobalDataPool* global_data_pool);
  Tensor Query(const Tensor& feats, const Tensor& dirs) override;
  Tensor QueryFromField(const Tensor& field_feats, const Tensor& dirs, const Tensor& app_emb, const Tensor& sample_emb_idx,
                        Tensor* app_emb_grad);
  Tensor SHEncode(const Tensor& dirs);
  std::vector<Tensor> States() override;
  std::vector<ParamGroup> OptimParamGroups() override;
  int LoadStates(const std::vector<Tensor>& states, int idx) override;
  void Reset() override;

  std::unique_ptr<FusedMLP> mlp_;
  int d_hidden_, n_hiddens_, degree_;
  bool fused_ok_ = true;
};

struct RenderResult {
  Tensor colors;
// ... 158 lines not shown
    pend_[i].s.counts_ready.synchronize();
    if (!pend_[i].s.completed && side_[i]) side_[i]->synchronize();
    pend_[i] = PendingBatch();
  }
  void DropPendingSamples() {
    for (int i = 0; i < kPendingSlots; i++) DropPendingSlot(i);
  }
  void KeepOnlyPending(const Tensor& o0, const Tensor& d0, const Tensor& o1, const Tensor& d1, const Tensor& o2, const Tensor& d2) {
    for (int i = 0; i < kPendingSlots; i++) {
      if (!pend_[i].s.active) continue;
      const int a = FindPending(o0, d0), b = FindPending(o1, d1), c = FindPending(o2, d2);
      if (i != a && i != b && i != c) DropPendingSlot(i);
    }
  }
  std::function<void()> after_octree_update_;
  int speculative_sampling_ = 2;
  static constexpr int kSpecQuietEpochs = 8;
  struct NextBatch {
    Tensor rays_o, rays_d;
    float fineness = 1.f;
    int64_t seq = -1;
    bool valid = false;
  } next_batch_, next2_batch_;
  int spec_depth_ = 2;
  int64_t n_speculative_ = 0, n_spec_fallback_ = 0;
  void PreSampleSpecBegin(int slot, const Tensor& rays_o, const Tensor& rays_d, float fineness, int64_t seq);
  void SpecBeginAtStepEnd();
  bool PreSampleSpecComplete(int slot);
  at::cuda::CUDAEvent spec_start_ev_;
  bool spec_start_recorded_ = false;
  c10::hip::HIPStreamMasqueradingAsCUDA* BeginDraw();
  void EndDraw();
  void ConsumedBehindStep(uint64_t seq_before);
  uint64_t ConsumedSeq() { return side_shared_ ? side_shared_->seq : 0; }
  at::cuda::CUDAEvent draw_ev_;
  bool draw_ev_recorded_ = false;
  bool rays_off_main_ = false;
  bool spec_start_is_consumed_ = false;
  RenderFront SampleAndFilter(const Tensor& rays_o, const Tensor& rays_d, const Tensor& bounds, const Tensor& emb_idx,
                              bool async_count = false);
  void ResolvePendingCount();
  int dp_world_ = 1;
  Tensor dp_count_, dp_count_host_;
  int dp_count_rays_ = 0, dp_sum_rays_ = 0;
  bool dp_sum_mirrored_ = false;
  at::cuda::CUDAEvent dp_count_ev_;
  float KeptPerRayForEma(int n_kept_local, int n_rays);
  static constexpr int kEmaRing = 32;
  struct EmaMark {
    int64_t seq = -1;
    float value = 0.f;
  } ema_ring_[kEmaRing];
  void RecordEma(int64_t seq) {
    if (seq >= 0) ema_ring_[seq % kEmaRing] = {seq, global_data_pool_->meaningful_sampled_pts_per_ray_};
  }
  bool EmaAfter(int64_t seq, float* value) const {
    if (seq < 0 || ema_ring_[seq % kEmaRing].seq != seq) return false;
    *value = ema_ring_[seq % kEmaRing].value;
    return true;
  }
  int64_t pending_count_seq_ = -1;
  static constexpr int kDigestRing = 32768;
  struct StepDigest {
    int64_t seq = -1;
    int iter = 0, n_rays = 0, n_marched = 0, n_kept = -1;
  };
  std::vector<StepDigest> digest_;
  void DigestBegin(int n_rays, int n_marched) {
    if (cur_seq_ < 0) return;
    if (digest_.empty()) digest_.resize(kDigestRing);
    digest_[cur_seq_ % kDigestRing] = {cur_seq_, global_data_pool_->iter_step_, n_rays, n_marched, -1};
  }
  void DigestKept(int64_t seq, int n_kept) {
    if (seq >= 0 && !digest_.empty() && digest_[seq % kDigestRing].seq == seq) digest_[seq % kDigestRing].n_kept = n_kept;
  }
  enum { TAP_PTS, TAP_DT, TAP_ANCHORS, TAP_F0, TAP_SURVIVORS, TAP_BG, TAP_EDGE, TAP_COLORS, TAP_TABLE_GRAD, TAP_SMALL_GRADS, TAP_TABLE,
         TAP_FIELD_MLP, TAP_COLOR_MLP, TAP_APP_EMB, TAP_GRAD_BEFORE, TAP_PTS_ALL_AFTER, TAP_VOL_ALL_AFTER, TAP_FIELD_X, TAP_DFEAT,
         TAP_PTS_PRE, TAP_DT_PRE, TAP_ANCHORS_PRE, TAP_PTS_ALL_PRE, TAP_VOL_ALL_PRE, N_TAPS };
  bool digest_taps_ = false;
  Tensor digest_tap_sums_;
  void DigestTap(int tap, const Tensor& t);
  bool async_count_ = false;
  bool prepass_feat_reuse_ = true;
  bool keep_prepass_outputs_ = false;
  int64_t n_feat_reuse_steps_ = 0;
  bool count_pending_ = false;
  int pending_count_rays_ = 0;
  int64_t total_kept_pts_ = 0, total_all_pts_ = 0;
  TrainOutputs TrainForwardBackward(const Tensor& rays_o, const Tensor& rays_d, const Tensor& bounds, const Tensor& gt_colors,
                                    const Tensor& emb_idx, float var_w, float disp_w, float tv_w);

  Tensor QueryDensity(const Tensor& world);
  Tensor DensityGrid(const std::vector<float>& lo, const std::vector<float>& hi, int res);
  std::tuple<Tensor, Tensor> ExtractMesh(const std::vector<float>& lo, const std::vector<float>& hi, int res, float level);
  static GridSpec MakeGridSpec(const std::vector<float>& lo, const std::vector<float>& hi, int res);
  Tensor DensityOfLocated(const Tensor& warped, const Tensor& anchors);
  std::tuple<Tensor, Tensor> QueryRadiance(const Tensor& world, const Tensor& dirs);
  MeshAttrs ExtractMeshAttrs(const std::vector<float>& lo, const std::vector<float>& hi, int res, float level, int min_component_faces,
                             bool normals, bool colors, const std::string& normal_source = "grid", int simplify = 0,
                             const MeshRefineOptions& refine = MeshRefineOptions());
  LevelProjection ProjectToLevel(const Tensor& points, float level, int iters, float max_step, float max_move, float tol,
                                 const Tensor& origins = Tensor());
  std::tuple<Tensor, Tensor> QueryDensityGrad(const Tensor& world);
  Tensor FieldNormals(const Tensor& world);
  void DensityGradSlabs(const Tensor& world, const Tensor& density, const Tensor& grad, const Tensor& normals);
  void DensityGradChunk(const Tensor& world, const Tensor& density, const Tensor& grad, const Tensor& normals);
  GeometryResult RenderGeometry(const Tensor& rays_o, const Tensor& rays_d, const Tensor& bounds, float tau, bool keep_samples);
  int64_t density_slab_points_ = int64_t(1) << 22;

  int LoadStates(const std::vector<Tensor>& states, int idx) override;
  std::vector<Tensor> States() override;
  std::vector<ParamGroup> OptimParamGroups() override;
  void ZeroGrad();
  bool FusedPathOk() const;

  GlobalDataPool* global_data_pool_;
  std::unique_ptr<PtsSampler> pts_sampler_;
  std::unique_ptr<Field> scene_field_;
  std::unique_ptr<Shader> shader_;
  bool use_app_emb_;
  Tensor app_emb_;
  Tensor app_emb_grad_;
  Tensor small_grads_flat_;
  BGColorType bg_color_type_ = BGColorType::rand_noise;
  SampleResultFlex sample_result_, presampled_;
  bool has_presample_ = false, presample_async_ = false;
  int presample_slot_ = 0;
  Tensor presample_rays_o_, presample_rays_d_;
  bool PresampleMatches(const Tensor& rays_o, const Tensor& rays_d) const;
  at::cuda::CUDAEvent octree_ready_ev_, presample_done_ev_[kPendingSlots], n_kept_ev_;
  at::cuda::CUDAEvent* kept_wait_ev_ = &n_kept_ev_;
  struct SideShared {
    std::shared_ptr<c10::hip::HIPStreamMasqueradingAsCUDA> stream[kPendingSlots];
    std::shared_ptr<c10::hip::HIPStreamMasqueradingAsCUDA> tail;
    at::cuda::CUDAEvent consumed;
    uint64_t seq = 0, waited[kPendingSlots] = {0, 0};
  };
  std::shared_ptr<SideShared> side_shared_;
  bool consumed_side_samples_ = false;
  void SideWaitConsumed(int slot);
  bool small_grads_clean_ = false;
  std::function<void()> after_count_readback_;
  std::function<bool(F2nStepTail*)> step_tail_builder_;
  bool TwoDeepRegime();
  std::function<void()> before_backward_;
  bool step_tail_done_ = false;
  c10::hip::HIPStreamMasqueradingAsCUDA* TailStream();
  MappedWords n_kept_words_;
  std::shared_ptr<c10::hip::HIPStreamMasqueradingAsCUDA> side_[kPendingSlots];
  void EnsureSideStream(int slot);
  Tensor forced_bg_;
  int n_edge_pts_ = 8192;
  int last_n_all_pts_ = 0, last_n_kept_pts_ = 0;
};

namespace CustomOps {
Tensor WeightVar(Tensor weights, Tensor idx_start_end);
}

}
```

f2-nerf_amd/csrc/host/RendererQuery.cpp:

```cpp
#include <cmath>
#include <limits>

#include "Renderer.h"

namespace f2n {

namespace {

Tensor Points3(const Tensor& t) {
  Tensor p = t.to(torch::kCUDA, torch::kFloat32).contiguous().view({-1, 3});
  TORCH_CHECK(p.size(0) <= INT32_MAX, "too many points");
  return p;
}

struct LocatedRows {
  Tensor se, total, pts, vol, src;
  int m = 0;
  LocatedRows(const Tensor& warped, const Tensor& anchors, bool want_src) {
    const int64_t n = anchors.size(0);
    Tensor counts = torch::empty({n}, DevI32());
    se = torch::empty({n, 2}, DevI32());
    total = torch::empty({1}, DevI32());
    Tensor cpts = torch::empty({n, 3}, DevF32()), cvol = torch::empty({n}, DevI32()), csrc;
    if (want_src) csrc = torch::empty({n}, DevI32());
    F2N_CALL(f2n_located_compact(CurStream(), (int) n, I32P(anchors), F32P(warped), I32P(counts), I32P(se), I32P(total), F32P(cpts),
                                 I32P(cvol), want_src ? I32P(csrc) : nullptr));
    m = total.item<int>();
    pts = cpts.narrow(0, 0, m);
    vol = cvol.narrow(0, 0, m);
    if (want_src) src = csrc.narrow(0, 0, m);
  }
};

struct PrepassCacheGuard {
  Hash3DAnchored* field;
  Tensor kept, kept_feat_h;
  explicit PrepassCacheGuard(Hash3DAnchored* f) : field(f), kept(f->prepass_x_), kept_feat_h(f->prepass_feat_h_) {}
  ~PrepassCacheGuard() {
    field->prepass_x_ = kept;
    field->prepass_feat_h_ = kept_feat_h;
  }
};

void Df0Dw(Hash3DAnchored* field, const Tensor& p, const Tensor& v, const Tensor& x_h, Tensor& g) {
  if (x_h.defined()) return field->DensityGrad(p, v, x_h, g);
  auto& mlp = *field->mlp_;
  const int m = (int) p.size(0);
  Tensor x = field->HashEncode(p, v).to(torch::kFloat32).contiguous();
  Tensor dy = torch::zeros({m, F2N_MLP_OUT_PAD}, DevF32());
  dy.select(1, 0).fill_(1.f);
  Tensor dparams = torch::zeros({mlp.n_params_}, DevF32()), dx = torch::empty({m, mlp.d_in_}, DevF32());
  F2N_CALL(f2n_mlp_bwd(CurStream(), m, mlp.d_in_, mlp.d_hidden_, mlp.n_hidden_layers_, 1.f, VoidP(mlp.params_h_), F32P(x), F32P(dy),
                       F32P(dparams), F32P(dx)));
  field->PosGrad(p, v, dx, g);
}

std::pair<int64_t, int64_t> TwoTotals(const Tensor& totals) {
  Tensor t = totals.cpu();
  return {t.data_ptr<int32_t>()[0], t.data_ptr<int32_t>()[1]};
}

}

std::tuple<Tensor, Tensor> PersSampler::LocatePoints(const Tensor& world) {
  torch::NoGradGuard g;
  Tensor w = Points3(world);
  const int64_t n = w.size(0);
  Tensor warped = torch::empty({n, 3}, DevF32()), anchors = torch::empty({n, 3}, DevI32());
  auto& o = *pers_octree_;
  F2N_CALL(f2n_oct_locate_warp(CurStream(), (int) n, F32P(w), VoidP(o.tree_nodes_gpu_), VoidP(o.pers_trans_gpu_), F32P(warped),
                               I32P(anchors)));
  return {warped, anchors};
}

Tensor Renderer::DensityOfLocated(const Tensor& warped, const Tensor& anchors) {
  torch::NoGradGuard g;
  auto* field = static_cast<Hash3DAnchored*>(scene_field_.get());
  const int64_t n = anchors.size(0);
  Tensor density = torch::empty({n}, DevF32());
  if (n == 0) return density;
  LocatedRows rows(warped, anchors, false);
  Tensor f0 = torch::zeros({1}, DevF32());
  if (rows.m > 0) {
    PrepassCacheGuard cache(field);
    f0 = field->QueryDensityPreAct(rows.pts, rows.vol, false);
  }
  F2N_CALL(f2n_density_scatter(CurStream(), (int) n, I32P(anchors), I32P(rows.se), F32P(f0), F32P(density)));
  return density;
}

Tensor Renderer::QueryDensity(const Tensor& world) {
  auto* sampler = static_cast<PersSampler*>(pts_sampler_.get());
  auto located = sampler->LocatePoints(world);
  return DensityOfLocated(std::get<0>(located), std::get<1>(located));
}

std::tuple<Tensor, Tensor> Renderer::QueryRadiance(const Tensor& world, const Tensor& dirs) {
  torch::NoGradGuard g;
  auto* sampler = static_cast<PersSampler*>(pts_sampler_.get());
  auto* field = static_cast<Hash3DAnchored*>(scene_field_.get());
  auto* shader = static_cast<SHShader*>(shader_.get());
  auto located = sampler->LocatePoints(world);
  const Tensor& warped = std::get<0>(located);
  const Tensor& anchors = std::get<1>(located);
  const int64_t n = anchors.size(0);
  Tensor d = Points3(dirs);
  TORCH_CHECK(d.size(0) == n, "one view direction per point");
  Tensor density = torch::empty({n}, DevF32()), rgb = torch::empty({n, 3}, DevF32());
  if (n == 0) return {density, rgb};
  LocatedRows rows(warped, anchors, true);
  const int m = rows.m;
  Tensor f0 = torch::zeros({1}, DevF32()), crgb = torch::zeros({1, 3}, DevF32());
  if (m > 0) {
    PrepassCacheGuard cache(field);
    Tensor cdirs = d.index_select(0, rows.src).contiguous();
    if (FusedPathOk()) {
      f0 = field->QueryDensityPreAct(rows.pts, rows.vol, true);
      TORCH_CHECK(field->prepass_x_.defined(), "no pre-pass feature cache for this query");
      crgb = torch::empty({m, 3}, DevF32());
      Tensor f0_again = torch::empty({m}, DevF32());
      F2N_CALL(f2n_field_shade_fwd_dyn(CurStream(), m, I32P(rows.total), nullptr, VoidP(field->prepass_x_), VoidP(field->mlp_->params_h_),
                                       F32P(cdirs), nullptr, nullptr, VoidP(shader->mlp_->params_h_), F32P(f0_again), nullptr, nullptr,
                                       F32P(crgb)));
// ... 937 lines not shown
```

f2-nerf_amd/csrc/host/RendererTrain.cpp:

```cpp
#include "Renderer.h"

#include <hip/hip_runtime_api.h>

#include <cstdio>
#include <cstdlib>
#include <mutex>

namespace f2n {

using torch::autograd::AutogradContext;
using torch::autograd::variable_list;

TrainOutputs Renderer::TrainForwardBackward(const Tensor& rays_o, const Tensor& rays_d, const Tensor& bounds,
                                            const Tensor& gt_colors, const Tensor& emb_idx, float var_w, float disp_w, float tv_w) {
  auto* gdp = global_data_pool_;
  auto* field = static_cast<Hash3DAnchored*>(scene_field_.get());
  auto* shader = static_cast<SHShader*>(shader_.get());
  torch::NoGradGuard no_grad;
  const int n_rays = rays_o.size(0);
  Tensor gt = gt_colors.contiguous();
  CheckDev(gt, torch::kFloat32, "gt_colors");
  TORCH_CHECK(gt.numel() == (int64_t) n_rays * 3, "gt_colors must be [n_rays,3]");
  struct KeepOutputs {
    bool& flag;
    KeepOutputs(bool& f, bool on) : flag(f) { flag = on; }
    ~KeepOutputs() { flag = false; }
  };
  RenderFront fr;
  {
    KeepOutputs keep(keep_prepass_outputs_, async_count_ && prepass_feat_reuse_ && !digest_taps_);
    fr = SampleAndFilter(rays_o, rays_d, bounds, emb_idx, async_count_);
  }
  void* st = CurStream();
  TrainOutputs out;
  out.losses = torch::empty({8}, DevF32());
  if (fr.empty) {
    Tensor bg = fr.bg_color.contiguous();
    F2N_CALL(f2n_train_loss(st, n_rays, F32P(bg), F32P(gt), nullptr, nullptr, 0, 0, nullptr, 0.f, 0.f, 0.f, F32P(out.losses),
                            nullptr, nullptr, nullptr, nullptr));
    return out;
  }
  SampleResultFlex& es = fr.es;
  const int n_kept = fr.n_kept, n_edge = fr.n_edge, n = n_kept + 2 * n_edge;
  TORCH_CHECK(FusedPathOk(), "the untaped training step needs the shipped network shapes (ExpRunner::TrainStep takes the taped path otherwise)");

  const int64_t so = fr.dyn ? 2 * (int64_t) n_edge : 0, eo = fr.dyn ? 0 : n_kept;
  const int32_t* n_dev = fr.dyn ? I32P(fr.n_kept_dev) : nullptr;
  Tensor feat = torch::empty({fr.dyn ? std::max(2 * n_edge, 1) : n, F2N_MLP_OUT_PAD}, DevF32());
  const bool reuse = fr.dyn && field->prepass_feat_h_.defined() && field->prepass_x_.defined();
  const bool edges_ride = fr.dyn && n_edge > 0 && fr.edge_cache_row >= 0;
  Tensor field_x = torch::empty({reuse ? (edges_ride ? 0 : 2 * n_edge) : n, N_LEVELS * N_CHANNELS}, DevF16());
  Tensor x_cache, feat_h_cache;
  Tensor f0c = torch::empty({std::max(n_kept, 1)}, DevF32()), df0c = torch::empty({std::max(n_kept, 1)}, DevF32());
  Tensor rgb = torch::empty({std::max(n_kept, 1), 3}, DevF32()), shade_x = torch::empty({std::max(n_kept, 1), 32}, DevF16());
  Tensor app = fr.emb ? app_emb_ : Tensor();
  if (fr.dyn) {
    TORCH_CHECK(field->prepass_x_.defined(), "no pre-pass feature cache for this query");
    if (n_edge > 0 && !edges_ride)
      F2N_TIMED_CALL("field_fwd", f2n_field_fwd(st, 2 * n_edge, field->n_volumes_, VoidP(field->feat_pool_h_), I32P(field->prim_pool_),
                             I32P(field->feat_local_idx_), I32P(field->feat_local_size_), F32P(field->bias_pool_),
                             F32P(field->level_scale_), F32P(fr.pts_all), I32P(fr.vol_all), 1, VoidP(field->mlp_->params_h_),
                             F32P(feat), nullptr, VoidP(field_x)));
    const at::Half* cache = field->prepass_x_.data_ptr<at::Half>();
    const int64_t row = (int64_t) N_LEVELS * N_CHANNELS;
    if (reuse) {
      x_cache = field->prepass_x_;
      feat_h_cache = field->prepass_feat_h_;
      n_feat_reuse_steps_++;
      const at::Half* fh = feat_h_cache.data_ptr<at::Half>();
      F2N_TIMED_CALL("field_shade_fwd", f2n_shade_fwd_feat(st, n_kept, n_dev, I32P(fr.src_rows),
                             static_cast<const void*>(fh + (int64_t) F2N_MLP_OUT_PAD * fr.sample_cache_row), F32P(es.dirs),
                             fr.emb ? F32P(app) : nullptr, fr.emb ? I32P(fr.sample_emb_idx) : nullptr, VoidP(shader->mlp_->params_h_),
                             F32P(f0c), VoidP(shade_x), F32P(rgb), edges_ride ? 2 * n_edge : 0,
                             edges_ride ? static_cast<const void*>(fh + (int64_t) F2N_MLP_OUT_PAD * fr.edge_cache_row) : nullptr,
                             edges_ride ? F32P(feat) : nullptr));
    } else {
      F2N_TIMED_CALL("field_shade_fwd", f2n_field_shade_fwd_extra(st, n_kept, n_dev, I32P(fr.src_rows),
                             static_cast<const void*>(cache + row * fr.sample_cache_row), VoidP(field->mlp_->params_h_), F32P(es.dirs),
                             fr.emb ? F32P(app) : nullptr, fr.emb ? I32P(fr.sample_emb_idx) : nullptr, VoidP(shader->mlp_->params_h_),
                             F32P(f0c), static_cast<void*>(field_x.data_ptr<at::Half>() + row * so), VoidP(shade_x), F32P(rgb),
                             edges_ride ? 2 * n_edge : 0, edges_ride ? static_cast<const void*>(cache + row * fr.edge_cache_row) : nullptr,
                             edges_ride ? F32P(feat) : nullptr, edges_ride ? VoidP(field_x) : nullptr));
    }
    field->DropPrepassCache();
  } else {
    field->ForwardRaw(fr.pts_all, fr.vol_all, 1, fr.src_rows, n_kept, feat, field_x, &f0c);
    field->DropPrepassCache();
    F2N_TIMED_CALL("shade_fwd", f2n_shade_fwd(st, n_kept, F32P(feat), F32P(es.dirs), fr.emb ? F32P(app) : nullptr,
                           fr.emb ? I32P(fr.sample_emb_idx) : nullptr, VoidP(shader->mlp_->params_h_), F32P(rgb), VoidP(shade_x)));
  }
  if (before_backward_) before_backward_();
  Tensor colors = torch::empty({n_rays, 3}, DevF32());
  Tensor weights = torch::empty({std::max(n_kept, 1)}, DevF32());
  Tensor bg = fr.bg_color.contiguous();
  Tensor dfeat = torch::empty({n, F2N_MLP_OUT_PAD}, DevF32());
  Tensor drgb = torch::empty({std::max(n_kept, 1), 3}, DevF32());
  if (fr.dyn) {
    F2N_TIMED_CALL("composite_train", f2n_composite_train(st, n_rays, I32P(es.pts_idx_bounds), F32P(f0c), 1, F32P(es.dt), F32P(es.t), F32P(rgb),
                                 F32P(bg), F32P(gt), var_w, disp_w, tv_w, gdp->gradient_scaling_progress_, n_edge, F2N_MLP_OUT_PAD,
                                 n_edge > 0 ? F32P(feat) + F2N_MLP_OUT_PAD * eo : nullptr, n_edge > 0 ? F32P(dfeat) + F2N_MLP_OUT_PAD * eo : nullptr,
                                 F32P(colors), F32P(weights), F32P(drgb), F32P(df0c), 1, F32P(out.losses), 1));
  } else {
    Tensor disparity = torch::empty({n_rays}, DevF32()), depth = torch::empty({n_rays}, DevF32());
    Tensor var = torch::empty({n_rays}, DevF32());
    F2N_TIMED_CALL("composite_fwd", f2n_composite_fwd(st, n_rays, I32P(es.pts_idx_bounds), F32P(f0c), 1, F32P(es.dt), F32P(es.t), F32P(rgb),
                               F32P(bg), F32P(colors), F32P(disparity), F32P(depth), F32P(weights), F32P(var)));

    Tensor dcolors = torch::empty({n_rays, 3}, DevF32()), ddisp = torch::empty({n_rays}, DevF32()), dvar = torch::empty({n_rays}, DevF32());
    F2N_TIMED_CALL("train_loss", f2n_train_loss(st, n_rays, F32P(colors), F32P(gt), F32P(disparity), F32P(var), n_edge, F2N_MLP_OUT_PAD,
                            F32P(feat) + F2N_MLP_OUT_PAD * eo, var_w, disp_w, tv_w, F32P(out.losses), F32P(dcolors),
                            F32P(ddisp), F32P(dvar), F32P(dfeat) + F2N_MLP_OUT_PAD * eo));

    F2N_TIMED_CALL("composite_bwd", f2n_composite_bwd(st, n_rays, I32P(es.pts_idx_bounds), F32P(f0c), 1, F32P(es.dt), F32P(es.t), F32P(rgb), F32P(bg),
                               F32P(dcolors), F32P(ddisp), nullptr, nullptr, gdp->gradient_scaling_progress_, F32P(drgb),
                               F32P(df0c), 1, F32P(weights), F32P(dvar)));
  }
  if (digest_taps_) DigestTap(TAP_GRAD_BEFORE, field->grad_h_);
  F2N_TIMED_CALL("shade_bwd", f2n_shade_bwd_dyn(st, n_kept, n_dev, F32P(drgb), fr.emb ? I32P(fr.sample_emb_idx) : nullptr,
                         VoidP(shader->mlp_->params_h_), VoidP(shade_x), shader->mlp_->loss_scale_, F32P(dfeat) + F2N_MLP_OUT_PAD * so,
                         F32P(shader->mlp_->grad_scaled_), fr.emb ? F32P(app_emb_grad_) : nullptr,
                         fr.emb ? (int) app_emb_grad_.size(0) : 0, F32P(df0c), fr.dyn ? 1 : 0));
  if (digest_taps_ && fr.dyn) {
    const int64_t rows = fr.pts_all.size(0);
    Tensor live = torch::arange(rows, DevI32()).lt(fr.n_kept_dev + (int) so).to(torch::kInt32);
    DigestTap(TAP_PTS_ALL_PRE, fr.pts_all.view(torch::kInt32).sum(1, false, torch::kInt64) * live);
    DigestTap(TAP_VOL_ALL_PRE, fr.vol_all.to(torch::kInt64) * live);
  }
  F2nStepTail tail;
  const bool fused_tail = fr.dyn && step_tail_builder_ && !digest_taps_ && step_tail_builder_(&tail);
  const int64_t xrow = (int64_t) N_LEVELS * N_CHANNELS;
  const void* x_edge = !reuse || n_edge == 0 ? nullptr
                       : edges_ride ? static_cast<const void*>(x_cache.data_ptr<at::Half>() + xrow * fr.edge_cache_row) : VoidP(field_x);
  const void* x_surv = reuse ? static_cast<const void*>(x_cache.data_ptr<at::Half>() + xrow * fr.sample_cache_row) : nullptr;
  if (fused_tail && reuse) {
    field->grad_clean_ = false;
    F2N_TIMED_CALL("field_bwd", f2n_field_bwd_step_tail_rows(st, TailStream()->stream(), n, n_dev, 2 * n_edge, field->n_volumes_, I32P(field->prim_pool_),
                           I32P(field->feat_local_idx_), I32P(field->feat_local_size_), F32P(field->bias_pool_),
                           F32P(field->level_scale_), F32P(fr.pts_all), I32P(fr.vol_all), 1, VoidP(field->mlp_->params_h_),
                           x_edge, x_surv, I32P(fr.src_rows), F32P(dfeat), field->mlp_->loss_scale_, F32P(field->mlp_->grad_scaled_),
                           VoidP(field->grad_h_), field->pool_size_ / N_LEVELS, &tail, nullptr));
    step_tail_done_ = true;
  } else if (fused_tail) {
    field->grad_clean_ = false;
    F2N_TIMED_CALL("field_bwd", f2n_field_bwd_step_tail(st, TailStream()->stream(), n, n_dev, 2 * n_edge, field->n_volumes_, I32P(field->prim_pool_),
                           I32P(field->feat_local_idx_), I32P(field->feat_local_size_), F32P(field->bias_pool_),
                           F32P(field->level_scale_), F32P(fr.pts_all), I32P(fr.vol_all), 1, VoidP(field->mlp_->params_h_),
                           VoidP(field_x), F32P(dfeat), field->mlp_->loss_scale_, F32P(field->mlp_->grad_scaled_),
                           VoidP(field->grad_h_), field->pool_size_ / N_LEVELS, &tail, nullptr));
    step_tail_done_ = true;
  } else if (reuse) {
    field->grad_clean_ = false;
    F2N_TIMED_CALL("field_bwd", f2n_field_bwd_dyn_rows(st, n, n_dev, 2 * n_edge, field->n_volumes_, I32P(field->prim_pool_),
                           I32P(field->feat_local_idx_), I32P(field->feat_local_size_), F32P(field->bias_pool_),
                           F32P(field->level_scale_), F32P(fr.pts_all), I32P(fr.vol_all), 1, VoidP(field->mlp_->params_h_),
                           x_edge, x_surv, I32P(fr.src_rows), F32P(dfeat), field->mlp_->loss_scale_, F32P(field->mlp_->grad_scaled_),
                           VoidP(field->grad_h_), field->pool_size_ / N_LEVELS, 1));
    F2N_TIMED_CALL("reduce_partials", f2n_reduce_deferred(st));
  } else if (fr.dyn) {
    field->grad_clean_ = false;
    F2N_TIMED_CALL("field_bwd", f2n_field_bwd_dyn(st, n, n_dev, 2 * n_edge, field->n_volumes_, I32P(field->prim_pool_),
                           I32P(field->feat_local_idx_), I32P(field->feat_local_size_), F32P(field->bias_pool_),
                           F32P(field->level_scale_), F32P(fr.pts_all), I32P(fr.vol_all), 1, VoidP(field->mlp_->params_h_),
                           VoidP(field_x), F32P(dfeat), field->mlp_->loss_scale_, F32P(field->mlp_->grad_scaled_),
                           VoidP(field->grad_h_), field->pool_size_ / N_LEVELS, 1));
    F2N_TIMED_CALL("reduce_partials", f2n_reduce_deferred(st));
  } else {
    field->BackwardRaw(fr.pts_all, fr.vol_all, 1, field_x, dfeat);
  }
  if (digest_taps_ && fr.dyn) {
    const int64_t rows = fr.pts_all.size(0);
    Tensor live = torch::arange(rows, DevI32()).lt(fr.n_kept_dev + (int) so).to(torch::kInt32);
    DigestTap(TAP_PTS_ALL_AFTER, fr.pts_all.view(torch::kInt32).sum(1, false, torch::kInt64) * live);
    DigestTap(TAP_VOL_ALL_AFTER, fr.vol_all.to(torch::kInt64) * live);
    Tensor live_n = live.narrow(0, 0, n);
    DigestTap(TAP_FIELD_X, field_x.view(torch::kInt32).sum(1, false, torch::kInt64) * live_n);
    DigestTap(TAP_DFEAT, dfeat.view(torch::kInt32).sum(1, false, torch::kInt64) * live_n);
  }
  if (digest_taps_) {
    DigestTap(TAP_COLORS, colors);
    DigestTap(TAP_TABLE_GRAD, field->grad_h_);
    DigestTap(TAP_SMALL_GRADS, small_grads_flat_);
  }
  if ((fr.side_pool_buffers || fr.consumed_deferred) && side_shared_) {
    side_shared_->consumed.record();
    side_shared_->seq++;
  }
  out.colors = colors;
  out.has_samples = true;
  return out;
}

}
```

f2-nerf_amd/csrc/host/bindings.cpp:

```cpp
#include <torch/extension.h>

#include "DataParallel.h"
#include "ExpRunner.h"

#include <hip/hip_runtime_api.h>

#include <algorithm>

using namespace f2n;

namespace {

Hash3DAnchored* FieldOf(ExpRunner& r) { return static_cast<Hash3DAnchored*>(r.renderer_->scene_field_.get()); }
SHShader* ShaderOf(ExpRunner& r) { return static_cast<SHShader*>(r.renderer_->shader_.get()); }
PersSampler* SamplerOf(ExpRunner& r) { return static_cast<PersSampler*>(r.renderer_->pts_sampler_.get()); }

struct InferenceMode {
  GlobalDataPool* gdp;
  RunningMode prev;
  InferenceMode(ExpRunner& r, bool on) : gdp(r.global_data_pool_.get()), prev(gdp->mode_) {
    if (on) gdp->mode_ = RunningMode::VALIDATE;
  }
  ~InferenceMode() { gdp->mode_ = prev; }
};
// ... 352 lines not shown
             d["iterations"] = n;
             d["total_meaningful"] = r.last_train_meaningful_;
             d["total_marched"] = r.last_train_marched_;
             d["total_rays"] = r.last_train_rays_;
             return d;
           },
           py::arg("dataset"), py::arg("until_iter") = -1, py::arg("sets") = DATA_TRAIN_SET)
      .def("render_train",
           [](ExpRunner& r, const Tensor& ro, const Tensor& rd, const Tensor& b, const Tensor& emb) {
             r.global_data_pool_->mode_ = RunningMode::TRAIN;
             auto rr = r.renderer_->Render(ro, rd, b, emb);
             py::dict d;
             d["colors"] = rr.colors; d["first_oct_dis"] = rr.first_oct_dis; d["disparity"] = rr.disparity;
             d["edge_feats"] = rr.edge_feats; d["depth"] = rr.depth; d["weights"] = rr.weights;
             d["idx_start_end"] = rr.idx_start_end;
             return d;
           })
      .def("get_samples",
           [](ExpRunner& r, const Tensor& ro, const Tensor& rd, const Tensor& b) {
             auto s = r.renderer_->pts_sampler_->GetSamples(ro, rd, b);
             py::dict d;
             d["pts"] = s.pts; d["dirs"] = s.dirs; d["dt"] = s.dt; d["t"] = s.t; d["anchors"] = s.anchors;
             d["pts_idx_bounds"] = s.pts_idx_bounds; d["first_oct_dis"] = s.first_oct_dis;
             return d;
           })
      .def("anchored_query", [](ExpRunner& r, const Tensor& pts, const Tensor& anchors) { return r.renderer_->scene_field_->AnchoredQuery(pts, anchors); })
      .def("shader_query", [](ExpRunner& r, const Tensor& feats, const Tensor& dirs) { return r.renderer_->shader_->Query(feats, dirs); })
      .def("zero_grad", [](ExpRunner& r) { r.renderer_->ZeroGrad(); })
      .def("optim_step", [](ExpRunner& r) { r.OptimStep(nullptr); })
      .def("grads",
           [](ExpRunner& r) {
             py::dict d;
             d["feat_pool"] = FieldOf(r)->TableGradUnscaled();
             d["field_mlp"] = FieldOf(r)->mlp_->GradUnscaled();
             d["color_mlp"] = ShaderOf(r)->mlp_->GradUnscaled();
             d["app_emb"] = r.renderer_->app_emb_grad_.clone();
             return d;
           })
      .def("grad_buffers",
           [](ExpRunner& r) {
             return std::vector<Tensor>{FieldOf(r)->grad_h_, FieldOf(r)->mlp_->grad_scaled_, ShaderOf(r)->mlp_->grad_scaled_,
                                        r.renderer_->app_emb_grad_};
           })
      .def("flatten_small_grads", &ExpRunner::FlattenSmallGrads)
      .def("occupancy_buffers",
           [](ExpRunner& r) {
             auto& o = *SamplerOf(r)->pers_octree_;
             return std::vector<Tensor>{o.tree_weight_stats_, o.tree_alpha_stats_, o.tree_visit_cnt_};
           })
      .def("set_grad_sync_hook", [](ExpRunner& r, py::function f) { r.sync_.blocking = [f]() { py::gil_scoped_acquire g; f(); }; })
      .def("set_pipelined_grad_sync",
           [](ExpRunner& r, py::function begin, py::function end) {
             r.sync_.begin = [begin]() { py::gil_scoped_acquire g; begin(); };
             r.sync_.end = [end]() { py::gil_scoped_acquire g; end(); };
             r.sync_.pipelined = true;
           })
      .def("flush", [](ExpRunner& r) { py::gil_scoped_release no_gil; r.FinishPending(); })
      .def("locate_points",
           [](ExpRunner& r, const Tensor& world) {
             py::gil_scoped_release no_gil;
             r.FinishPending();
             auto t = SamplerOf(r)->LocatePoints(world);
             return std::vector<Tensor>{std::get<0>(t), std::get<1>(t)};
           })
      .def("query_density",
           [](ExpRunner& r, const Tensor& world) {
             py::gil_scoped_release no_gil;
             r.FinishPending();
             return r.renderer_->QueryDensity(world);
           })
      .def("density_prepass",
           [](ExpRunner& r, const Tensor& warped, const Tensor& anchors, bool keep_outputs) {
             py::gil_scoped_release no_gil;
             r.FinishPending();
             return FieldOf(r)->QueryDensityPreAct(warped, anchors, true, keep_outputs);
           },
           py::arg("warped"), py::arg("anchors"), py::arg("keep_outputs") = true)
      .def("prepass_caches",
           [](ExpRunner& r) {
             auto* f = FieldOf(r);
             Tensor none = torch::empty({0}, torch::kFloat16);
             return std::vector<Tensor>{f->prepass_x_.defined() ? f->prepass_x_ : none, f->prepass_feat_h_.defined() ? f->prepass_feat_h_ : none};
           })
      .def("density_grid",
           [](ExpRunner& r, const std::vector<float>& lo, const std::vector<float>& hi, int res) {
             py::gil_scoped_release no_gil;
             r.FinishPending();
             return r.renderer_->DensityGrid(lo, hi, res);
           },
           py::arg("lo"), py::arg("hi"), py::arg("res"))
      .def("extract_mesh",
           [](ExpRunner& r, const std::vector<float>& lo, const std::vector<float>& hi, int res, float level) {
             py::gil_scoped_release no_gil;
             r.FinishPending();
             auto t = r.renderer_->ExtractMesh(lo, hi, res, level);
             return std::vector<Tensor>{std::get<0>(t), std::get<1>(t)};
           },
           py::arg("lo"), py::arg("hi"), py::arg("res"), py::arg("level"))
      .def("query_radiance",
           [](ExpRunner& r, const Tensor& world, const Tensor& dirs) {
             py::gil_scoped_release no_gil;
             r.FinishPending();
             auto t = r.renderer_->QueryRadiance(world, dirs);
             return std::vector<Tensor>{std::get<0>(t), std::get<1>(t)};
           },
           py::arg("world"), py::arg("dirs"))
      .def("extract_mesh_attrs",
           [](ExpRunner& r, const std::vector<float>& lo, const std::vector<float>& hi, int res, float level, int min_component_faces,
              bool normals, bool colors, const std::string& normal_source, int simplify, const py::object& refine) {
             MeshRefineOptions ro;
             if (!refine.is_none()) {
               ro.on = true;
               for (auto item : refine.cast<py::dict>()) {
                 const std::string key = item.first.cast<std::string>();
                 if (key == "smooth_passes") ro.smooth_passes = item.second.cast<int>();
                 else if (key == "lam") ro.lam = item.second.cast<double>();
                 else if (key == "mu") ro.mu = item.second.cast<double>();
                 else if (key == "project") ro.project = item.second.cast<bool>();
                 else if (key == "iters") ro.iters = item.second.cast<int>();
                 else if (key == "max_step_steps") ro.max_step_steps = item.second.cast<float>();
                 else if (key == "max_move_steps") ro.max_move_steps = item.second.cast<float>();
                 else if (key == "tol") ro.tol = item.second.cast<float>();
                 else throw std::invalid_argument("extract_mesh_attrs: unknown refine option \"" + key + "\"");
               }
             }
             MeshAttrs a;
             {
               py::gil_scoped_release no_gil;
               r.FinishPending();
               InferenceMode mode(r, ro.on);
               a = r.renderer_->ExtractMeshAttrs(lo, hi, res, level, min_component_faces, normals, colors, normal_source, simplify, ro);
             }
             py::dict d;
             d["verts"] = a.verts;
             d["faces"] = a.faces;
             if (normals) d["normals"] = a.normals;
             if (colors) d["colors"] = a.colors;
             if (simplify >= 2) {
               d["verts_in"] = a.verts_in;
               d["faces_in"] = a.faces_in;
             }
             if (ro.on) {
               py::dict s;
               for (const auto& kv : a.refine) {
                 const bool real = kv.first.rfind("h_", 0) == 0 || kv.first.rfind("moved_", 0) == 0 || kv.first.rfind("quality_", 0) == 0 ||
                                   kv.first.rfind("max_", 0) == 0;
                 if (real) s[py::str(kv.first)] = kv.second;
                 else s[py::str(kv.first)] = (int64_t) kv.second;
               }
               d["refine"] = s;
             }
             return d;
           },
           py::arg("lo"), py::arg("hi"), py::arg("res"), py::arg("level"), py::arg("min_component_faces") = 0, py::arg("normals") = true,
           py::arg("colors") = true, py::arg("normal_source") = "grid",
           py::arg("simplify") = 0,
           py::arg("refine") = py::none())
      .def("project_to_level",
           [](ExpRunner& r, const Tensor& points, float level, int iters, float max_step, float max_move, float tol,
              const c10::optional<Tensor>& origins) {
             LevelProjection p;
             {
               py::gil_scoped_release no_gil;
               r.FinishPending();
               InferenceMode mode(r, true);
               p = r.renderer_->ProjectToLevel(points, level, iters, max_step, max_move, tol, origins.has_value() ? *origins : Tensor());
// ... 86 lines not shown
                  [](int begin_us, int complete_us, int main_us, int period, unsigned pollute) {
                    Renderer::SetDebugSideDelay(begin_us, complete_us, main_us, period, pollute);
                  },
                  py::arg("begin_us"), py::arg("complete_us"), py::arg("main_us"), py::arg("period"), py::arg("pollute") = 0u)
#endif
      .def_static("enable_kernel_timing", [](const std::vector<std::string>& names) { KernelTimers::Get().Enable(names); })
      .def_static("disable_kernel_timing", []() { KernelTimers::Get().Disable(); })
      .def_static("collect_kernel_timing",
                  []() {
                    py::dict d;
                    for (auto& kv : KernelTimers::Get().Collect()) d[py::str(kv.first)] = py::make_tuple(kv.second.first, kv.second.second);
                    return d;
                  })
      .def("install_octree", [](ExpRunner& r, const Tensor& n, const Tensor& t, const Tensor& e) { SamplerOf(r)->InstallOctree(n, t, e); })
      .def("set_edge_pool",[](ExpRunner& r, const Tensor& e) { SamplerOf(r)->SetEdgePool(e); })
      .def("set_train_cameras", [](ExpRunner& r, const Tensor& w2c, const Tensor& intri, const Tensor& b) { SamplerOf(r)->SetTrainCameras(w2c, intri, b); })
      .def("set_forced_randoms",
           [](ExpRunner& r, const Tensor& noise, const Tensor& bg, const Tensor& edge_idx, const Tensor& edge_coords) {
             SamplerOf(r)->forced_noise_ = noise;
             r.renderer_->forced_bg_ = bg;
             SamplerOf(r)->forced_edge_idx_ = edge_idx;
             SamplerOf(r)->forced_edge_coords_ = edge_coords;
           })
      .def("clear_forced_randoms",
           [](ExpRunner& r) {
             SamplerOf(r)->forced_noise_ = Tensor(); r.renderer_->forced_bg_ = Tensor();
             SamplerOf(r)->forced_edge_idx_ = Tensor(); SamplerOf(r)->forced_edge_coords_ = Tensor();
           })
      .def("n_nodes", [](ExpRunner& r) { return SamplerOf(r)->pers_octree_->n_nodes_; })
      .def("proc_octree", [](ExpRunner& r, bool compact, bool subdivide, bool brute) { SamplerOf(r)->pers_octree_->ProcOctree(compact, subdivide, brute); })
      .def("tree_nodes", [](ExpRunner& r) { return SamplerOf(r)->pers_octree_->tree_nodes_gpu_; })
      .def("cur_batch_size", &ExpRunner::CurBatchSize)
      .def("batch_size_for", &ExpRunner::BatchSizeFor)
      .def_property("step_seq",
                    [](ExpRunner& r) { return r.step_seq_; }, [](ExpRunner& r, int64_t s) { r.ResetStepSequence(s); })
      .def_readwrite("digest_table", &ExpRunner::digest_table_)
      .def_property("digest_taps",
                    [](ExpRunner& r) { return r.renderer_->digest_taps_; }, [](ExpRunner& r, bool on) { r.renderer_->digest_taps_ = on; })
      .def("step_taps",
           [](ExpRunner& r) {
             r.FinishPending();
             std::vector<int64_t> seqs;
             for (auto& d : r.renderer_->digest_) if (d.seq >= 0) seqs.push_back(d.seq);
             std::sort(seqs.begin(), seqs.end());
             Tensor out = torch::zeros({(int64_t) seqs.size(), 1 + Renderer::N_TAPS}, torch::kInt64);
             if (!r.renderer_->digest_tap_sums_.defined()) return out;
             Tensor sums = r.renderer_->digest_tap_sums_.cpu();
             for (size_t i = 0; i < seqs.size(); i++) {
               out[i][0] = seqs[i];
               out[i].narrow(0, 1, Renderer::N_TAPS).copy_(sums[seqs[i] % Renderer::kDigestRing]);
             }
             return out;
           })
      .def("step_digest",
           [](ExpRunner& r) {
             r.FinishPending();
             py::list out;
             auto& dg = r.renderer_->digest_;
             Tensor sums = r.digest_table_sums_.defined() ? r.digest_table_sums_.cpu() : Tensor();
             std::vector<Renderer::StepDigest> rows;
             for (auto& d : dg) if (d.seq >= 0) rows.push_back(d);
             std::sort(rows.begin(), rows.end(), [](const Renderer::StepDigest& a, const Renderer::StepDigest& b) { return a.seq < b.seq; });
             for (auto& d : rows) {
               py::list row;
               row.append(d.seq); row.append(d.iter); row.append(d.n_rays); row.append(d.n_marched); row.append(d.n_kept);
               if (sums.defined()) row.append(sums.data_ptr<int64_t>()[d.seq % Renderer::kDigestRing]);
               out.append(row);
             }
             return out;
           })
      .def_readwrite("iter_step", &ExpRunner::iter_step_)
      .def_readwrite("check_nan", &ExpRunner::check_nan_)
      .def_readwrite("async_counts", &ExpRunner::async_counts_)
      .def_property("speculative_sampling",
                    [](ExpRunner& r) { return r.renderer_->speculative_sampling_; },
                    [](ExpRunner& r, int mode) { r.renderer_->speculative_sampling_ = mode; })
      .def_property("tail_repair",
                    [](ExpRunner& r) { return static_cast<PersSampler*>(r.renderer_->pts_sampler_.get())->tail_repair_; },
                    [](ExpRunner& r, bool on) { static_cast<PersSampler*>(r.renderer_->pts_sampler_.get())->tail_repair_ = on; })
      .def_readwrite("fused_tail", &ExpRunner::fused_tail_)
      .def_property("prepass_feat_reuse",
                    [](ExpRunner& r) { return r.renderer_->prepass_feat_reuse_; },
                    [](ExpRunner& r, bool on) { r.renderer_->prepass_feat_reuse_ = on; })
      .def_property_readonly("prepass_reuse_steps", [](ExpRunner& r) { return r.renderer_->n_feat_reuse_steps_; })
      .def_readwrite("spec_start_without_event", &ExpRunner::spec_start_without_event_)
      .def_readwrite("draws_off_main", &ExpRunner::draws_off_main_)
      .def_readwrite("exact_flag_order", &ExpRunner::exact_flag_order_)
      .def_property("march_block_waves",
                    [](ExpRunner& r) { return static_cast<PersSampler*>(r.renderer_->pts_sampler_.get())->march_block_waves_; },
                    [](ExpRunner& r, int n) { static_cast<PersSampler*>(r.renderer_->pts_sampler_.get())->march_block_waves_ = std::min(16, std::max(1, n)); })
      .def_property("march_blocks",
                    [](ExpRunner& r) { return static_cast<PersSampler*>(r.renderer_->pts_sampler_.get())->march_blocks_; },
                    [](ExpRunner& r, int n) { static_cast<PersSampler*>(r.renderer_->pts_sampler_.get())->march_blocks_ = std::max(0, n); })
      .def_property("speculation_depth",
                    [](ExpRunner& r) { return r.renderer_->spec_depth_; },
                    [](ExpRunner& r, int d) { r.FinishPending(); r.renderer_->DropPendingSamples(); r.renderer_->spec_depth_ = std::max(1, std::min(3, d)); })
      .def("speculation_counters",
           [](ExpRunner& r) {
             r.FinishPending();
             py::dict d;
             d["speculative"] = r.renderer_->n_speculative_;
             d["fallback"] = r.renderer_->n_spec_fallback_;
             d["dropped"] = r.renderer_->n_spec_dropped_;
             auto& o = *SamplerOf(r)->pers_octree_;
             d["rays_repaired"] = o.n_repaired_.defined() ? o.n_repaired_.item<int>() : 0;
             d["stat_updates"] = o.epoch_;
             return d;
           })
      .def("counters",
           [](ExpRunner& r) {
             r.FinishPending();
             py::dict d;
             d["total_meaningful"] = r.renderer_->total_kept_pts_;
             d["total_marched"] = r.renderer_->total_all_pts_;
             return d;
           })
      .def_readonly("cur_lr", &ExpRunner::cur_lr_)
      .def_property("n_edge_pts", [](ExpRunner& r) { return r.renderer_->n_edge_pts_; }, [](ExpRunner& r, int n) { r.renderer_->n_edge_pts_ = n; })
      .def_property_readonly("fineness", [](ExpRunner& r) { return r.global_data_pool_->ray_march_fineness_; })
      .def_property_readonly("oct_per_ray", [](ExpRunner& r) { return r.global_data_pool_->sampled_oct_per_ray_; })
      .def_property_readonly("sampled_per_ray", [](ExpRunner& r) { return r.global_data_pool_->sampled_pts_per_ray_; })
      .def_property_readonly("meaningful_per_ray", [](ExpRunner& r) { return r.global_data_pool_->meaningful_sampled_pts_per_ray_; })
      .def_property_readonly("n_volumes", [](ExpRunner& r) { return r.global_data_pool_->n_volumes_; })
      .def("update_ada_params", &ExpRunner::UpdateAdaParams);
}
```

include/f2n_abi.h:

```cpp
#ifndef F2N_ABI_H
#define F2N_ABI_H

#include <stdint.h>

#ifdef __cplusplus
extern "C" {
#endif

#define F2N_OK 0
#define F2N_ERR_INVALID_ARG (-1)
#define F2N_ERR_UNSUPPORTED (-2)

#define F2N_N_LEVELS 16
#define F2N_N_CHANNELS 2
#define F2N_MAX_SAMPLE_PER_RAY 1024
#define F2N_MLP_OUT_PAD 16

int f2n_abi_version(void);
int f2n_numerics_mode(void);
const char* f2n_build_info(void);
typedef void (*f2n_bucket_fn)(void* user, int bucket, int n_buckets);
int f2n_set_scatter_buckets(int n_buckets, f2n_bucket_fn fn, void* user);
int f2n_set_scatter_buckets_for(int n_buckets, f2n_bucket_fn fn, void* user, const void* grad_table_h16);
int f2n_debug_counters(int32_t* out8_host , int reset);
// ... 281 lines not shown
                       float* gt_colors , float* bounds);
int f2n_draw_ray_batch_keyed(void* stream, int n_rays, uint64_t key, uint64_t seq, const int32_t* image_set, int n_set, int height,
                             int width, const float* poses, const float* intri, const float* dist_params, const float* images ,
                             const float* cam_bounds, int32_t* cam_indices, int32_t* ij, float* rays_o, float* rays_d,
                             float* gt_colors , float* bounds);

int f2n_adam_coefficients(int step, float lr, double beta1, double beta2, float eps, float weight_decay, float grad_scale,
                          float* out9 );
int f2n_adam_step(void* stream, int n, float* param, float* grad, float grad_scale, int grad_round_h16,
                  float* exp_avg, float* exp_avg_sq, int step, float lr, double beta1, double beta2, float eps,
                  float weight_decay, void* param_h_or_null, int zero_grad ,
                  const int32_t* skip_flag );
typedef struct F2nAdamGroup {
  float* param;
  float* grad;
  float* exp_avg;
  float* exp_avg_sq;
  void* param_h;
  int n;
  float grad_scale;
  float weight_decay;
  int grad_round_h16;
  int check_finite;
} F2nAdamGroup;
int f2n_adam_small_groups(void* stream, int n_groups, const F2nAdamGroup* groups, int step, float lr, double beta1,
                          double beta2, float eps, int zero_grad, int32_t* flags ,
                          const int32_t* skip_flag );
int f2n_adam_fused(void* stream, int n_groups, const F2nAdamGroup* groups, int n_table, float* table_param, void* table_grad_h,
                   float table_grad_scale, float* table_exp_avg, float* table_exp_avg_sq, void* table_param_h, int step, float lr,
                   double beta1, double beta2, float eps, int zero_grad, const int32_t* skip_flag );
typedef struct F2nStepTail {
  int n_flags_a;
  const float* flags_grad_a;
  int n_flags_b;
  const float* flags_grad_b;
  int32_t* flags;
  int32_t* flags_mirror;
  int n_groups;
  const F2nAdamGroup* groups;
  int n_table;
  float* table_param;
  float* table_exp_avg;
  float* table_exp_avg_sq;
  void* table_param_h;
  float table_grad_scale;
  int step;
  float lr;
  double beta1, beta2;
  float eps;
  void (*after_reduce)(void* user, void* chain_stream);
  void* after_reduce_user;
  int leave_table_to_caller;
} F2nStepTail;
int f2n_field_bwd_step_tail(void* stream, void* tail_stream , int n_max, const int32_t* n_dev, int n_off, int n_volumes,
                            const int32_t* prim_pool, const int32_t* local_idx, const int32_t* local_size, const float* bias_pool,
                            const float* level_scale, const float* pts_warped, const int32_t* volume_idx, int vol_stride,
                            const void* mlp_params_h, const void* saved_x_h, const float* dfeat, float loss_scale,
                            float* dparams_f32_scaled, void* grad_table_h, int level_entries, const F2nStepTail* tail,
                            int* table_stepped_by_owners );
int f2n_field_fwd_ex(void* stream, int n, int n_volumes, const void* table_h, const int32_t* prim_pool,
                     const int32_t* local_idx, const int32_t* local_size, const float* bias_pool,
                     const float* level_scale, const float* pts_warped, const int32_t* volume_idx, int vol_stride,
                     const void* mlp_params_h, float* out_feat_f32, float* out_f0, void* save_x_h, void* out_feat_h);
int f2n_field_fwd_fused_ex(void* stream, int n, int n_volumes, const void* table_h, const int32_t* prim_pool, const int32_t* local_idx,
                           const int32_t* local_size, const float* bias_pool, const float* level_scale, const float* pts_warped,
                           const int32_t* volume_idx, int vol_stride, const void* mlp_params_h, float* out_feat_f32 ,
                           float* out_f0 , void* save_x_h , void* out_feat_h );
int f2n_field_mlp_planes_ex(void* stream, int n, const void* planes_h, const void* mlp_params_h, float* out_feat_f32,
                            float* out_f0, void* save_x_h, void* out_feat_h);
int f2n_shade_fwd_feat(void* stream, int n_max, const int32_t* n_dev, const int32_t* src_rows, const void* feat_cache_h,
                       const float* dirs, const float* app_emb, const int32_t* sample_emb_idx, const void* color_params_h,
                       float* out_f0, void* save_shade_x_h, float* rgb, int n_extra, const void* feat_extra_h, float* feat_extra);
int f2n_field_bwd_dyn_rows(void* stream, int n_max, const int32_t* n_dev, int n_off, int n_volumes, const int32_t* prim_pool,
                           const int32_t* local_idx, const int32_t* local_size, const float* bias_pool, const float* level_scale,
                           const float* pts_warped, const int32_t* volume_idx, int vol_stride, const void* mlp_params_h,
                           const void* x_edge_h, const void* x_cache_h, const int32_t* src_rows, const float* dfeat, float loss_scale,
                           float* dparams_f32_scaled, void* grad_table_h, int level_entries, int defer_reduce);
int f2n_field_bwd_step_tail_rows(void* stream, void* tail_stream , int n_max, const int32_t* n_dev, int n_off, int n_volumes,
                                 const int32_t* prim_pool, const int32_t* local_idx, const int32_t* local_size, const float* bias_pool,
                                 const float* level_scale, const float* pts_warped, const int32_t* volume_idx, int vol_stride,
                                 const void* mlp_params_h, const void* x_edge_h, const void* x_cache_h, const int32_t* src_rows,
                                 const float* dfeat, float loss_scale, float* dparams_f32_scaled, void* grad_table_h, int level_entries,
                                 const F2nStepTail* tail, int* table_stepped_by_owners );
int f2n_adam_step_h16grad(void* stream, int n, float* param, void* grad_h, float grad_scale, float* exp_avg,
                          float* exp_avg_sq, int step, float lr, double beta1, double beta2, float eps,
                          float weight_decay, void* param_h, int zero_grad, const int32_t* skip_flag );

int f2n_train_loss(void* stream, int n_rays, const float* pred_colors , const float* gt_colors ,
                   const float* disparity , const float* sampled_var , int n_edge, int feat_dim,
                   const float* edge_feats , float var_w, float disp_w, float tv_w,
                   float* out_losses , float* dcolors, float* ddisparity, float* dvar, float* dedge_feats);

int f2n_composite_train(void* stream, int n_rays, const int32_t* pts_start_end, const float* f0, int f0_stride, const float* dt,
                        const float* t, const float* rgb, const float* bg, const float* gt_colors, float var_w, float disp_w, float tv_w,
                        float grad_scaling_progress, int n_edge, int feat_dim, const float* edge_feats ,
                        float* dedge_feats , float* colors, float* weights, float* drgb, float* df0, int df0_stride,
                        float* out_losses , int defer_reduce);

int f2n_nonfinite_flags(void* stream, int n_a, const float* a, int n_b, const float* b, int32_t* flags );
int f2n_nonfinite_flags_ex(void* stream, int n_a, const float* a, int n_b, const float* b, int32_t* flags ,
                           int32_t* mirror );

int f2n_oct_locate_warp(void* stream, int n, const float* pts_world , const void* tree_nodes, const void* transes,
                        float* out_pts_warped , int32_t* out_anchors );
int f2n_oct_locate_warp_grid(void* stream, const float* lo , float step, int nx, int ny, int nz, int first_z, int n_z,
                             const void* tree_nodes, const void* transes, float* out_pts_warped ,
                             int32_t* out_anchors );
int f2n_located_compact(void* stream, int n, const int32_t* anchors , const float* pts_warped , int32_t* counts ,
                        int32_t* start_end , int32_t* total , float* out_pts , int32_t* out_vol ,
                        int32_t* out_src );
int f2n_density_scatter(void* stream, int n, const int32_t* anchors , const int32_t* start_end , const float* f0,
                        float* density );
int f2n_mesh_count(void* stream, int nx, int ny, int nz, const float* grid, float level, uint8_t* edge_mask ,
                   int32_t* vert_counts , int32_t* vert_start_end , int32_t* face_counts ,
                   int32_t* face_start_end , int32_t* totals );
int f2n_mesh_emit(void* stream, int nx, int ny, int nz, const float* grid, float level, const float* lo , float step,
                  const uint8_t* edge_mask, const int32_t* vert_start_end, const int32_t* face_start_end, float* verts, int32_t* faces);
int f2n_radiance_scatter(void* stream, int n, const int32_t* anchors , const int32_t* start_end , const float* f0,
                         const float* rgb_rows, float* density , float* rgb );
int f2n_grid_normals(void* stream, int n, const float* pts , const float* grid, int nx, int ny, int nz,
                     const float* lo , float step, float* out );
int f2n_mesh_components(void* stream, int n_verts, int n_faces, const int32_t* faces , int32_t* labels ,
                        int32_t* changed , int* rounds );
int f2n_mesh_filter_count(void* stream, int n_verts, int n_faces, const int32_t* faces , const int32_t* labels ,
                          int min_faces, int32_t* comp_faces , int32_t* vert_keep , int32_t* vert_start_end ,
                          int32_t* face_keep , int32_t* face_start_end , int32_t* totals );
int f2n_mesh_filter_emit(void* stream, int n_verts, int n_faces, const float* verts , const int32_t* faces ,
                         const int32_t* vert_keep, const int32_t* vert_start_end, const int32_t* face_keep, const int32_t* face_start_end,
                         float* out_verts, int32_t* vert_src, int32_t* out_faces);
int f2n_field_density_grad(void* stream, int n, int n_volumes, const void* table_h, const int32_t* prim_pool, const int32_t* local_idx,
                           const int32_t* local_size, const float* bias_pool, const float* level_scale, const float* pts_warped,
                           const int32_t* volume_idx, int vol_stride, const void* mlp_params_h, const void* x_h ,
                           float* out_dx , float* out_df0_dw );
int f2n_hash_pos_grad(void* stream, int n, int n_volumes, const void* table_h, const int32_t* prim_pool, const int32_t* local_idx,
                      const int32_t* local_size, const float* bias_pool, const float* level_scale, const float* pts_warped,
                      const int32_t* volume_idx, int vol_stride, const float* dx , float* out_df0_dw );
int f2n_density_grad_scatter(void* stream, int n, const float* pts_world , const int32_t* anchors ,
                             const int32_t* start_end , const void* transes, const float* f0, const float* df0_dw ,
                             float* out_density , float* out_grad , float* out_normal );

int f2n_composite_geometry(void* stream, int n_rays, const int32_t* pts_start_end , const float* weights ,
                           const float* t , const float* rays_o , const float* rays_d ,
                           const int32_t* anchors , const void* transes, const float* df0_dw , float tau,
                           float* out_opacity , float* out_normal , int32_t* out_surf_idx , float* out_surf_t ,
                           float* out_surf_point , float* out_surf_normal , float* out_sample_grad ,
                           float* out_sample_normal );

int f2n_tsdf_integrate(void* stream, const float* lo , float step, int nx, int ny, int nz, int n_views,
                       const float* poses , const float* intri , const float* dist_params ,
                       const float* depth , const float* conf , int h, int w, float trunc,
                       float* S , float* W );
int f2n_tsdf_finalize(void* stream, int64_t n, const float* S, const float* W, float min_weight, float* g , uint8_t* valid );
int f2n_mesh_count_masked(void* stream, int nx, int ny, int nz, const float* grid, float level, const uint8_t* valid ,
                          uint8_t* edge_mask , int32_t* vert_counts , int32_t* vert_start_end ,
                          int32_t* face_counts , int32_t* face_start_end , int32_t* totals );

int f2n_mesh_cluster_keys(void* stream, int n_verts, const float* verts , const float* lo , float cell,
                          const int32_t* dims , int64_t* keys );
int f2n_mesh_cluster_accumulate(void* stream, int n_verts, int n_faces, const float* verts , const int32_t* faces ,
                                const int32_t* cluster_of , int n_clusters, const float* lo , float cell,
                                const int32_t* dims , int64_t* acc , int32_t* flag );
int f2n_mesh_cluster_place(void* stream, int n_clusters, const int64_t* acc , const int64_t* cluster_keys ,
                           const float* lo , float cell, const int32_t* dims , double lambda,
                           float* out_verts );
int f2n_mesh_cluster_faces(void* stream, int n_verts, int n_faces, const int32_t* faces , const int32_t* cluster_of ,
                           int32_t* out_faces );
// ... 67 lines not shown
```

Measured before the change: 695.7 million ray-samples/s.

## Add planar-layout prepass cache path for field MLP forward and backward

Adds a plane-major (channel-group-strided) layout for the cached prepass encoding, along with a dedicated MLP forward kernel that reads those planes with prefetching. New backward kernels and step-tail entry points read the encoded inputs from the planes, including edge samples. This is meant to make the per-lane fragment loads contiguous and coalesced instead of strided row gathers. The path sits behind a new prepass_planes_cache flag and adds ABI surface and more kernel template instantiations.

```diff
diff --git a/f2-nerf_amd/capi.py b/f2-nerf_amd/capi.py
--- a/f2-nerf_amd/capi.py
+++ b/f2-nerf_amd/capi.py
@@ -640,6 +640,17 @@
                                      _i(int(defer_reduce))), "f2n_field_bwd_dyn_rows")
 
 
+def field_bwd_dyn_planes(n_max, n_dev, n_off, n_volumes, prim_pool, local_idx, local_size, bias_pool, level_scale, pts_warped, volume_idx,
+                         vol_stride, mlp_params_h, x_edge_h, x_edge_planes_h, x_planes_h, plane_rows, src_rows, dfeat, loss_scale,
+                         dparams_scaled, grad_table_h, level_entries, defer_reduce):
+    _ck(lib().f2n_field_bwd_dyn_planes(_stream(), _i(n_max), _p(n_dev, "i32", True), _i(n_off), _i(n_volumes), _p(prim_pool, "i32"),
+                                       _p(local_idx, "i32"), _p(local_size, "i32"), _p(bias_pool, "f32"), _p(level_scale, "f32"),
+                                       _p(pts_warped, "f32"), _p(volume_idx, "i32"), _i(vol_stride), _p(mlp_params_h, "h16"),
+                                       _p(x_edge_h, "h16", True), _p(x_edge_planes_h, "h16", True), _p(x_planes_h, "h16"), _i(plane_rows),
+                                       _p(src_rows, "i32"), _p(dfeat, "f32"), _f(loss_scale), _p(dparams_scaled, "f32"),
+                                       _p(grad_table_h, "h16"), _i(level_entries), _i(int(defer_reduce))), "f2n_field_bwd_dyn_planes")
+
+
 class _StepTail(ctypes.Structure):
     _fields_ = [("n_flags_a", ctypes.c_int), ("flags_grad_a", ctypes.c_void_p), ("n_flags_b", ctypes.c_int), ("flags_grad_b", ctypes.c_void_p),
                 ("flags", ctypes.c_void_p), ("flags_mirror", ctypes.c_void_p), ("n_groups", ctypes.c_int), ("groups", ctypes.c_void_p),
@@ -652,7 +663,7 @@
 def field_bwd_step_tail(n_max, n_dev, n_off, n_volumes, prim_pool, local_idx, local_size, bias_pool, level_scale, pts_warped, volume_idx,
                         vol_stride, mlp_params_h, saved_x_h, dfeat, loss_scale, dparams_scaled, grad_table_h, level_entries, flags_a,
                         flags_b, flags, groups, table, step, lr, beta1, beta2, eps, tail_stream=None, flags_mirror=None, leave_table_to_caller=False,
-                        after_reduce=None, x_cache_h=None, src_rows=None):
+                        after_reduce=None, x_cache_h=None, src_rows=None, plane_rows=0, x_edge_planes_h=None):
     arr = (_AdamGroup * max(len(groups), 1))()
     for a, g in zip(arr, groups):
         a.param = _p(g["param"], "f32").value
@@ -681,6 +692,15 @@
         t.after_reduce = ctypes.cast(cb, ctypes.c_void_p).value
     by_owners = ctypes.c_int(0)
     ts = ctypes.c_void_p(tail_stream.cuda_stream) if tail_stream is not None else ctypes.c_void_p(0)
+    if plane_rows > 0:
+        _ck(lib().f2n_field_bwd_step_tail_planes(_stream(), ts, _i(n_max), _p(n_dev, "i32", True), _i(n_off), _i(n_volumes), _p(prim_pool, "i32"),
+                                                 _p(local_idx, "i32"), _p(local_size, "i32"), _p(bias_pool, "f32"), _p(level_scale, "f32"),
+                                                 _p(pts_warped, "f32"), _p(volume_idx, "i32"), _i(vol_stride), _p(mlp_params_h, "h16"),
+                                                 _p(saved_x_h, "h16", True), _p(x_edge_planes_h, "h16", True), _p(x_cache_h, "h16"),
+                                                 _i(plane_rows), _p(src_rows, "i32"), _p(dfeat, "f32"), _f(loss_scale),
+                                                 _p(dparams_scaled, "f32"), _p(grad_table_h, "h16"), _i(level_entries), ctypes.byref(t),
+                                                 ctypes.byref(by_owners)), "f2n_field_bwd_step_tail_planes")
+        return by_owners.value
     if x_cache_h is not None:
         _ck(lib().f2n_field_bwd_step_tail_rows(_stream(), ts, _i(n_max), _p(n_dev, "i32", True), _i(n_off), _i(n_volumes), _p(prim_pool, "i32"),
                                                _p(local_idx, "i32"), _p(local_size, "i32"), _p(bias_pool, "f32"), _p(level_scale, "f32"),
diff --git a/f2-nerf_amd/csrc/field.hip b/f2-nerf_amd/csrc/field.hip
--- a/f2-nerf_amd/csrc/field.hip
+++ b/f2-nerf_amd/csrc/field.hip
@@ -1065,6 +1065,48 @@
   }
 }
 
+__global__ __launch_bounds__(F2N_FWD_THREADS) void field_mlp_planes_kernel(int n, const half_t* __restrict__ params,
+                                                                           const half_t* __restrict__ x_planes,
+                                                                           float* __restrict__ out_feat_f32, half_t* __restrict__ out_feat_h,
+                                                                           float* __restrict__ out_f0, half_t* __restrict__ save_x) {
+  F2N_RAISE_PRIO();
+  const int tid = threadIdx.x, lane = tid & 63, c = lane & 15, g = lane >> 4;
+  F2nMlpFwdW<1> w;
+  w.load(params, c, g);
+  const int n_tiles = (n + 15) / 16;
+  const int wave_global = blockIdx.x * (F2N_FWD_THREADS / 64) + (tid >> 6);
+  const int wave_stride = gridDim.x * (F2N_FWD_THREADS / 64);
+  auto fetch = [&](int tile) {
+    const int s = tile * 16 + c;
+    const int sc = s < n ? s : n - 1;
+    return f2n_cat(*(const half4_t*) (x_planes + ((size_t) g * n + sc) * 4), *(const half4_t*) (x_planes + ((size_t) (4 + g) * n + sc) * 4));
+  };
+  if (wave_global >= n_tiles) return;
+  half8_t cur = fetch(wave_global);
+  for (int tile = wave_global; tile < n_tiles; tile += wave_stride) {
+    const half8_t nxt = fetch(tile + wave_stride < n_tiles ? tile + wave_stride : tile);
+    __builtin_amdgcn_sched_barrier(0);
+    const int s = tile * 16 + c;
+    const bool valid = s < n;
+    const half8_t xf = valid ? cur : half8_t{0, 0, 0, 0, 0, 0, 0, 0};
+    if (save_x != nullptr && valid) f2n_store_xfrag_h(save_x, s, g, xf);
+    const float4_t o = w.forward(xf);
+    if (valid) {
+      half4_t oh;
+      float4_t of;
+#pragma unroll
+      for (int r = 0; r < 4; r++) {
+        oh[r] = (half_t) o[r];
+        of[r] = (float) oh[r];
+      }
+      if (out_feat_f32 != nullptr) *(float4_t*) (out_feat_f32 + (size_t) s * F2N_D_OUT + 4 * g) = of;
+      if (out_feat_h != nullptr) *(half4_t*) (out_feat_h + (size_t) s * F2N_D_OUT + 4 * g) = oh;
+      if (out_f0 != nullptr && g == 0) out_f0[s] = of[0];
+    }
+    cur = nxt;
+  }
+}
+
 #define F2N_BWD_THREADS 256
 
 template <int NH>
@@ -1073,7 +1115,10 @@
   float acc[2 * (F2N_D_HID * F2N_D_IN + (NH == 2 ? F2N_D_HID * F2N_D_HID : 0) + F2N_D_OUT * F2N_D_HID)];
 };
 
-template <int NH, int HASH, bool ROWS>
+#define F2N_X_COMPACT 0
+#define F2N_X_ROWS 1
+#define F2N_X_PLANES 2
+template <int NH, int HASH, int SRC>
 __device__ __forceinline__ void f2n_field_bwd_body(
     int n, F2nHashArgs h, const int32_t* __restrict__ local_idx, const int32_t* __restrict__ local_size,
     const float* __restrict__ level_scale, const float* __restrict__ pts, int pts_are_warped,
@@ -1081,8 +1126,9 @@
     const half_t* __restrict__ x_h, const float* __restrict__ x_f32, const float* __restrict__ dy, float loss_scale,
     float* __restrict__ dparams, float* __restrict__ dx_f32, half_t* __restrict__ grad_table, half_t* __restrict__ dx_planes,
     uint16_t* __restrict__ nz_mask, const int32_t* __restrict__ n_dev, int n_off, const half_t* __restrict__ x_cache,
-    const int32_t* __restrict__ src_rows) {
+    const int32_t* __restrict__ src_rows, const half_t* __restrict__ x_edge_planes, int plane_rows) {
   F2N_RAISE_PRIO();
+  constexpr bool ROWS = SRC != F2N_X_COMPACT;
   const int n_alloc = n;
   if (n_dev != nullptr) n = min(n, *n_dev + n_off);
   __shared__ F2nBwdSmem<NH> sm;
@@ -1109,7 +1155,13 @@
   auto fetch = [&](int tile, int row, In& o) {
     const int s = tile * 16 + c;
     const int sc = s < n ? s : n - 1;
-    if (ROWS) o.xf = f2n_rowfrag(row >= 0 ? x_cache + (size_t) row * F2N_D_IN : x_h + (size_t) sc * F2N_D_IN, F2N_D_IN, 0, 0, g);
+    if (SRC == F2N_X_PLANES) {
+      const bool in_planes = row >= 0 || x_edge_planes != nullptr;
+      const half_t* p = row >= 0                   ? x_cache + ((size_t) g * plane_rows + row) * 4
+                        : x_edge_planes != nullptr ? x_edge_planes + ((size_t) g * plane_rows + sc) * 4
+                                                   : x_h + (size_t) sc * F2N_D_IN + 4 * g;
+      o.xf = f2n_cat(*(const half4_t*) p, *(const half4_t*) (p + (in_planes ? (size_t) 16 * plane_rows : (size_t) 16)));
+    } else if (ROWS) o.xf = f2n_rowfrag(row >= 0 ? x_cache + (size_t) row * F2N_D_IN : x_h + (size_t) sc * F2N_D_IN, F2N_D_IN, 0, 0, g);
     else o.xf = (x_h != nullptr) ? f2n_load_xfrag_h(x_h, sc, g, true) : f2n_load_xfrag_f32(x_f32, sc, g, true);
     o.d4 = *(const float4_t*) (dy + (size_t) sc * F2N_D_OUT + 4 * g);
   };
@@ -1189,9 +1241,9 @@
     const half_t* __restrict__ x_h, const float* __restrict__ x_f32, const float* __restrict__ dy, float loss_scale,
     float* __restrict__ dparams, float* __restrict__ dx_f32, half_t* __restrict__ grad_table, half_t* __restrict__ dx_planes,
     uint16_t* __restrict__ nz_mask, const int32_t* __restrict__ n_dev, int n_off) {
-  f2n_field_bwd_body<NH, HASH, false>(n, h, local_idx, local_size, level_scale, pts, pts_are_warped, volume_idx, vol_stride, params, x_h,
-                                      x_f32, dy, loss_scale, dparams, dx_f32, grad_table, dx_planes, nz_mask, n_dev, n_off, nullptr,
-                                      nullptr);
+  f2n_field_bwd_body<NH, HASH, F2N_X_COMPACT>(n, h, local_idx, local_size, level_scale, pts, pts_are_warped, volume_idx, vol_stride, params,
+                                              x_h, x_f32, dy, loss_scale, dparams, dx_f32, grad_table, dx_planes, nz_mask, n_dev, n_off,
+                                              nullptr, nullptr, nullptr, 0);
 }
 
 template <int HASH, int BPC>
@@ -1202,9 +1254,23 @@
     const half_t* __restrict__ x_edge, const half_t* __restrict__ x_cache, const int32_t* __restrict__ src_rows,
     const float* __restrict__ dy, float loss_scale, float* __restrict__ dparams, half_t* __restrict__ grad_table,
     half_t* __restrict__ dx_planes, uint16_t* __restrict__ nz_mask, const int32_t* __restrict__ n_dev, int n_off) {
-  f2n_field_bwd_body<1, HASH, true>(n, h, local_idx, local_size, level_scale, pts, pts_are_warped, volume_idx, vol_stride, params, x_edge,
-                                    nullptr, dy, loss_scale, dparams, nullptr, grad_table, dx_planes, nz_mask, n_dev, n_off, x_cache,
-                                    src_rows);
+  f2n_field_bwd_body<1, HASH, F2N_X_ROWS>(n, h, local_idx, local_size, level_scale, pts, pts_are_warped, volume_idx, vol_stride, params,
+                                          x_edge, nullptr, dy, loss_scale, dparams, nullptr, grad_table, dx_planes, nz_mask, n_dev, n_off,
+                                          x_cache, src_rows, nullptr, 0);
+}
+
+template <int HASH, int BPC>
+__global__ __launch_bounds__(F2N_BWD_THREADS, BPC) void field_bwd_planes_kernel(
+    int n, F2nHashArgs h, const int32_t* __restrict__ local_idx, const int32_t* __restrict__ local_size,
+    const float* __restrict__ level_scale, const float* __restrict__ pts, int pts_are_warped,
+    const int32_t* __restrict__ volume_idx, int vol_stride, const half_t* __restrict__ params,
+    const half_t* __restrict__ x_edge, const half_t* __restrict__ x_edge_planes, const half_t* __restrict__ x_planes, int plane_rows,
+    const int32_t* __restrict__ src_rows, const float* __restrict__ dy, float loss_scale, float* __restrict__ dparams,
+    half_t* __restrict__ grad_table, half_t* __restrict__ dx_planes, uint16_t* __restrict__ nz_mask, const int32_t* __restrict__ n_dev,
+    int n_off) {
+  f2n_field_bwd_body<1, HASH, F2N_X_PLANES>(n, h, local_idx, local_size, level_scale, pts, pts_are_warped, volume_idx, vol_stride, params,
+                                            x_edge, nullptr, dy, loss_scale, dparams, nullptr, grad_table, dx_planes, nz_mask, n_dev, n_off,
+                                            x_planes, src_rows, x_edge_planes, plane_rows);
 }
 
 __global__ __launch_bounds__(256) void hash_bwd_kernel(int n, F2nHashArgs h, const int32_t* __restrict__ local_idx,
@@ -1840,11 +1906,8 @@
                             void* save_x_h, void* out_feat_h) {
   if (n < 0 || (n > 0 && planes_h == nullptr)) return F2N_ERR_INVALID_ARG;
   if (n == 0) return F2N_OK;
-  F2nHashArgs h = {nullptr, nullptr, nullptr, 1};
-  hipLaunchKernelGGL((field_fwd_kernel<1, false, true>), dim3(f2n_wave_grid((n + 15) / 16, 4)), dim3(F2N_FWD_THREADS), 0,
-                     (hipStream_t) stream, n, h, nullptr, nullptr, nullptr, nullptr, 0, nullptr, 1, nullptr,
-                     (const half_t*) mlp_params_h, out_feat_f32, (half_t*) out_feat_h, out_f0, (half_t*) save_x_h, (const half_t*) planes_h,
-                     nullptr, nullptr, nullptr);
+  hipLaunchKernelGGL(field_mlp_planes_kernel, dim3(f2n_wave_grid((n + 15) / 16, 4)), dim3(F2N_FWD_THREADS), 0, (hipStream_t) stream, n,
+                     (const half_t*) mlp_params_h, (const half_t*) planes_h, out_feat_f32, (half_t*) out_feat_h, out_f0, (half_t*) save_x_h);
   return f2n_launch_status();
 }
 
@@ -1913,12 +1976,16 @@
                               const void* mlp_params_h, const void* saved_x_h, const float* dfeat, float loss_scale,
                               float* dparams_f32_scaled, void* grad_table_h, int level_entries, int defer_reduce,
                               const F2nStepTail* tail, int* table_stepped, const void* x_cache_h = nullptr,
-                              const int32_t* src_rows = nullptr) {
+                              const int32_t* src_rows = nullptr, const void* x_edge_planes_h = nullptr, int plane_rows = 0) {
   const int n = n_max;
   if (table_stepped != nullptr) *table_stepped = 0;
   if (n < 0 || n_volumes <= 0 || vol_stride < 1 || !(loss_scale > 0.f) || level_entries < 0 || ((uintptr_t) mlp_params_h & 15))
     return F2N_ERR_INVALID_ARG;
-  if (x_cache_h != nullptr && (src_rows == nullptr || n_off < 0 || n_off > n || (n_off > 0 && saved_x_h == nullptr))) return F2N_ERR_INVALID_ARG;
+  if (x_cache_h != nullptr && (src_rows == nullptr || n_off < 0 || n_off > n || (n_off > 0 && saved_x_h == nullptr && x_edge_planes_h == nullptr)))
+    return F2N_ERR_INVALID_ARG;
+  if (plane_rows < 0 || (plane_rows > 0 && (x_cache_h == nullptr || ((uintptr_t) x_cache_h & 7) || ((uintptr_t) x_edge_planes_h & 7))) ||
+      (plane_rows == 0 && x_edge_planes_h != nullptr))
+    return F2N_ERR_INVALID_ARG;
   if (tail != nullptr && (tail->flags == nullptr || tail->n_groups < 0 || tail->n_groups > 4 || tail->step < 1 || tail->n_table < 0 ||
                           (tail->n_table > 0 && (tail->table_param == nullptr || tail->table_exp_avg == nullptr ||
                                                  tail->table_exp_avg_sq == nullptr || tail->table_param_h == nullptr))))
@@ -1950,13 +2017,22 @@
                      local_idx, local_size, level_scale, pts_warped, 1, volume_idx, vol_stride, (const half_t*) mlp_params_h,  \
                      (const half_t*) saved_x_h, (const half_t*) x_cache_h, src_rows, dfeat, loss_scale, partials,             \
                      (half_t*) grad_table_h, dx_planes, nz_mask, n_dev, n_off)
-    if (x_cache_h != nullptr) {
+#define F2N_LAUNCH_FIELD_BWD_PLANES(HASH, BPC)                                                                                  \
+  hipLaunchKernelGGL((field_bwd_planes_kernel<HASH, BPC>), dim3(blocks), dim3(F2N_BWD_THREADS), 0, (hipStream_t) stream, n, h,  \
+                     local_idx, local_size, level_scale, pts_warped, 1, volume_idx, vol_stride, (const half_t*) mlp_params_h,   \
+                     (const half_t*) saved_x_h, (const half_t*) x_edge_planes_h, (const half_t*) x_cache_h, plane_rows, src_rows, \
+                     dfeat, loss_scale, partials, (half_t*) grad_table_h, dx_planes, nz_mask, n_dev, n_off)
+    if (plane_rows > 0) {
+      if (!bins) F2N_LAUNCH_FIELD_BWD_PLANES(1, 2);
+      else F2N_LAUNCH_FIELD_BWD_PLANES(2, 3);
+    } else if (x_cache_h != nullptr) {
       if (!bins) F2N_LAUNCH_FIELD_BWD_ROWS(1, 2);
       else F2N_LAUNCH_FIELD_BWD_ROWS(2, 3);
     } else if (!bins) F2N_LAUNCH_FIELD_BWD(1, 2);
     else F2N_LAUNCH_FIELD_BWD(2, 3);
 #undef F2N_LAUNCH_FIELD_BWD
 #undef F2N_LAUNCH_FIELD_BWD_ROWS
+#undef F2N_LAUNCH_FIELD_BWD_PLANES
     rc = f2n_launch_status();
     if (rc != F2N_OK) return rc;
     if (tail == nullptr && !defer_reduce) {
@@ -2073,4 +2149,28 @@
                             level_entries, 1, tail, table_stepped_by_owners, x_cache_h, src_rows);
 }
 
-}
+int f2n_field_bwd_dyn_planes(void* stream, int n_max, const int32_t* n_dev, int n_off, int n_volumes, const int32_t* prim_pool,
+                             const int32_t* local_idx, const int32_t* local_size, const float* bias_pool, const float* level_scale,
+                             const float* pts_warped, const int32_t* volume_idx, int vol_stride, const void* mlp_params_h,
+                             const void* x_edge_h, const void* x_edge_planes_h, const void* x_planes_h, int plane_rows,
+                             const int32_t* src_rows, const float* dfeat, float loss_scale, float* dparams_f32_scaled, void* grad_table_h,
+                             int level_entries, int defer_reduce) {
+  if (x_planes_h == nullptr || plane_rows < 1) return F2N_ERR_INVALID_ARG;
+  return f2n_field_bwd_impl(stream, nullptr, n_max, n_dev, n_off, n_volumes, prim_pool, local_idx, local_size, bias_pool, level_scale, pts_warped,
+                            volume_idx, vol_stride, mlp_params_h, x_edge_h, dfeat, loss_scale, dparams_f32_scaled, grad_table_h, level_entries,
+                            defer_reduce, nullptr, nullptr, x_planes_h, src_rows, x_edge_planes_h, plane_rows);
+}
+
+int f2n_field_bwd_step_tail_planes(void* stream, void* tail_stream, int n_max, const int32_t* n_dev, int n_off, int n_volumes,
+                                   const int32_t* prim_pool, const int32_t* local_idx, const int32_t* local_size, const float* bias_pool,
+                                   const float* level_scale, const float* pts_warped, const int32_t* volume_idx, int vol_stride,
+                                   const void* mlp_params_h, const void* x_edge_h, const void* x_edge_planes_h, const void* x_planes_h,
+                                   int plane_rows, const int32_t* src_rows, const float* dfeat, float loss_scale, float* dparams_f32_scaled,
+                                   void* grad_table_h, int level_entries, const F2nStepTail* tail, int* table_stepped_by_owners) {
+  if (tail == nullptr || x_planes_h == nullptr || plane_rows < 1) return F2N_ERR_INVALID_ARG;
+  return f2n_field_bwd_impl(stream, tail_stream, n_max, n_dev, n_off, n_volumes, prim_pool, local_idx, local_size, bias_pool, level_scale,
+                            pts_warped, volume_idx, vol_stride, mlp_params_h, x_edge_h, dfeat, loss_scale, dparams_f32_scaled, grad_table_h,
+                            level_entries, 1, tail, table_stepped_by_owners, x_planes_h, src_rows, x_edge_planes_h, plane_rows);
+}
+
+}
diff --git a/f2-nerf_amd/csrc/host/Field.cpp b/f2-nerf_amd/csrc/host/Field.cpp
--- a/f2-nerf_amd/csrc/host/Field.cpp
+++ b/f2-nerf_amd/csrc/host/Field.cpp
@@ -290,7 +290,8 @@
   return mlp_out_dim_ == F2N_MLP_OUT_PAD ? feat : feat.index({Slc(), Slc(0, mlp_out_dim_)}).contiguous();
 }
 
-Tensor Hash3DAnchored::QueryDensityPreAct(const Tensor& points, const Tensor& anchors, bool keep_features, bool keep_outputs) {
+Tensor Hash3DAnchored::QueryDensityPreAct(const Tensor& points, const Tensor& anchors, bool keep_features, bool keep_outputs,
+                                          bool keep_planes) {
   torch::NoGradGuard g;
   Tensor pts = points.contiguous();
   CheckDev(pts, torch::kFloat32, "points");
@@ -301,7 +302,7 @@
     return mlp_->Query(HashEncode(pts, anchors)).select(1, 0).contiguous();
   }
   Tensor f0 = torch::empty({n}, DevF32());
-  prepass_x_ = keep_features ? torch::empty({n, N_LEVELS * N_CHANNELS}, DevF16()) : Tensor();
+  prepass_planes_ = Tensor();
   prepass_feat_h_ = keep_features && keep_outputs ? torch::empty({n, F2N_MLP_OUT_PAD}, DevF16()) : Tensor();
   void* feat_h = prepass_feat_h_.defined() ? VoidP(prepass_feat_h_) : nullptr;
 #if F2N_DEBUG_BUILD
@@ -312,6 +313,8 @@
 #else
   constexpr bool force_fused = false;
 #endif
+  const bool planes_cache = keep_planes && keep_features && keep_outputs && !force_fused && n >= 32768;
+  prepass_x_ = keep_features && !planes_cache ? torch::empty({n, N_LEVELS * N_CHANNELS}, DevF16()) : Tensor();
   if (force_fused) {
     F2N_TIMED_CALL("field_prepass_fused", f2n_field_fwd_fused_ex(CurStream(), n, n_volumes_, VoidP(feat_pool_h_), I32P(prim_pool_),
                            I32P(feat_local_idx_), I32P(feat_local_size_), F32P(bias_pool_), F32P(level_scale_), F32P(pts), I32P(av.t),
@@ -343,7 +346,8 @@
                              I32P(av.t), av.stride, VoidP(planes), balance_gather_ ? step01 : 0.f, level_scale_host_.data()));
     }
     F2N_TIMED_CALL("field_mlp_prepass", f2n_field_mlp_planes_ex(CurStream(), n, VoidP(planes), VoidP(mlp_->params_h_), nullptr, F32P(f0),
-                           keep_features ? VoidP(prepass_x_) : nullptr, feat_h));
+                           prepass_x_.defined() ? VoidP(prepass_x_) : nullptr, feat_h));
+    if (planes_cache) prepass_planes_ = planes;
   } else {
     F2N_TIMED_CALL("field_prepass", f2n_field_fwd_ex(CurStream(), n, n_volumes_, VoidP(feat_pool_h_), I32P(prim_pool_), I32P(feat_local_idx_),
                            I32P(feat_local_size_), F32P(bias_pool_), F32P(level_scale_), F32P(pts), I32P(av.t), av.stride,
diff --git a/f2-nerf_amd/csrc/host/Hash3DAnchored.h b/f2-nerf_amd/csrc/host/Hash3DAnchored.h
--- a/f2-nerf_amd/csrc/host/Hash3DAnchored.h
+++ b/f2-nerf_amd/csrc/host/Hash3DAnchored.h
@@ -12,8 +12,9 @@
  public:
   explicit Hash3DAnchored(GlobalDataPool* global_data_pool);
   Tensor AnchoredQuery(const Tensor& points, const Tensor& anchors) override;
-  Tensor QueryDensityPreAct(const Tensor& points, const Tensor& anchors, bool keep_features = false, bool keep_outputs = false);
-  void DropPrepassCache() { prepass_x_ = Tensor(); prepass_feat_h_ = Tensor(); }
+  Tensor QueryDensityPreAct(const Tensor& points, const Tensor& anchors, bool keep_features = false, bool keep_outputs = false,
+                            bool keep_planes = false);
+  void DropPrepassCache() { prepass_x_ = Tensor(); prepass_feat_h_ = Tensor(); prepass_planes_ = Tensor(); }
   Tensor AnchoredQueryReuse(const Tensor& points, const Tensor& anchors, const Tensor& src_rows, int n_reuse);
   void ForwardRaw(const Tensor& points, const Tensor& anchors, int stride, const Tensor& src_rows, int n_reuse, Tensor& feat,
                   Tensor& saved_x, Tensor* f0_cached = nullptr);
@@ -42,6 +43,7 @@
   bool grad_clean_ = false;
   Tensor prepass_x_;
   Tensor prepass_feat_h_;
+  Tensor prepass_planes_;
   std::unique_ptr<FusedMLP> mlp_;
   int n_volumes_;
   std::vector<float> level_scale_host_;
diff --git a/f2-nerf_amd/csrc/host/Renderer.cpp b/f2-nerf_amd/csrc/host/Renderer.cpp
--- a/f2-nerf_amd/csrc/host/Renderer.cpp
+++ b/f2-nerf_amd/csrc/host/Renderer.cpp
@@ -327,7 +327,8 @@
         DigestTap(TAP_DT_PRE, sample_result_.dt);
         DigestTap(TAP_ANCHORS_PRE, sample_result_.anchors.select(1, 0));
       }
-      f0_full = field->QueryDensityPreAct(pts_full, anchors_full, true, keep_prepass_outputs_);
+      f0_full = field->QueryDensityPreAct(pts_full, anchors_full, true, keep_prepass_outputs_,
+                                          keep_prepass_outputs_ && prepass_planes_cache_);
       f0p = F32P(f0_full) + front;
       if (digest_taps_ && train) DigestTap(TAP_EDGE, pts_full.narrow(0, 0, front));
       fr.edge_cache_row = 0;
@@ -339,7 +340,8 @@
         DigestTap(TAP_DT_PRE, sample_result_.dt);
         DigestTap(TAP_ANCHORS_PRE, sample_result_.anchors.select(1, 0));
       }
-      f0_full = field->QueryDensityPreAct(sample_result_.pts, sample_result_.anchors, true, keep_prepass_outputs_);
+      f0_full = field->QueryDensityPreAct(sample_result_.pts, sample_result_.anchors, true, keep_prepass_outputs_,
+                                          keep_prepass_outputs_ && prepass_planes_cache_);
       f0p = F32P(f0_full);
     }
     if (digest_taps_ && train) {
diff --git a/f2-nerf_amd/csrc/host/Renderer.h b/f2-nerf_amd/csrc/host/Renderer.h
--- a/f2-nerf_amd/csrc/host/Renderer.h
+++ b/f2-nerf_amd/csrc/host/Renderer.h
@@ -264,6 +264,7 @@
   void DigestTap(int tap, const Tensor& t);
   bool async_count_ = false;
   bool prepass_feat_reuse_ = true;
+  bool prepass_planes_cache_ = true;
   bool keep_prepass_outputs_ = false;
   int64_t n_feat_reuse_steps_ = 0;
   bool count_pending_ = false;
diff --git a/f2-nerf_amd/csrc/host/RendererQuery.cpp b/f2-nerf_amd/csrc/host/RendererQuery.cpp
--- a/f2-nerf_amd/csrc/host/RendererQuery.cpp
+++ b/f2-nerf_amd/csrc/host/RendererQuery.cpp
@@ -34,11 +34,12 @@
 
 struct PrepassCacheGuard {
   Hash3DAnchored* field;
-  Tensor kept, kept_feat_h;
-  explicit PrepassCacheGuard(Hash3DAnchored* f) : field(f), kept(f->prepass_x_), kept_feat_h(f->prepass_feat_h_) {}
+  Tensor kept, kept_feat_h, kept_planes;
+  explicit PrepassCacheGuard(Hash3DAnchored* f) : field(f), kept(f->prepass_x_), kept_feat_h(f->prepass_feat_h_), kept_planes(f->prepass_planes_) {}
   ~PrepassCacheGuard() {
     field->prepass_x_ = kept;
     field->prepass_feat_h_ = kept_feat_h;
+    field->prepass_planes_ = kept_planes;
   }
 };
 
diff --git a/f2-nerf_amd/csrc/host/RendererTrain.cpp b/f2-nerf_amd/csrc/host/RendererTrain.cpp
--- a/f2-nerf_amd/csrc/host/RendererTrain.cpp
+++ b/f2-nerf_amd/csrc/host/RendererTrain.cpp
@@ -47,7 +47,8 @@
   const int64_t so = fr.dyn ? 2 * (int64_t) n_edge : 0, eo = fr.dyn ? 0 : n_kept;
   const int32_t* n_dev = fr.dyn ? I32P(fr.n_kept_dev) : nullptr;
   Tensor feat = torch::empty({fr.dyn ? std::max(2 * n_edge, 1) : n, F2N_MLP_OUT_PAD}, DevF32());
-  const bool reuse = fr.dyn && field->prepass_feat_h_.defined() && field->prepass_x_.defined();
+  const bool planes = fr.dyn && field->prepass_feat_h_.defined() && field->prepass_planes_.defined();
+  const bool reuse = fr.dyn && field->prepass_feat_h_.defined() && (field->prepass_x_.defined() || planes);
   const bool edges_ride = fr.dyn && n_edge > 0 && fr.edge_cache_row >= 0;
   Tensor field_x = torch::empty({reuse ? (edges_ride ? 0 : 2 * n_edge) : n, N_LEVELS * N_CHANNELS}, DevF16());
   Tensor x_cache, feat_h_cache;
@@ -55,16 +56,15 @@
   Tensor rgb = torch::empty({std::max(n_kept, 1), 3}, DevF32()), shade_x = torch::empty({std::max(n_kept, 1), 32}, DevF16());
   Tensor app = fr.emb ? app_emb_ : Tensor();
   if (fr.dyn) {
-    TORCH_CHECK(field->prepass_x_.defined(), "no pre-pass feature cache for this query");
+    TORCH_CHECK(field->prepass_x_.defined() || planes, "no pre-pass feature cache for this query");
     if (n_edge > 0 && !edges_ride)
       F2N_TIMED_CALL("field_fwd", f2n_field_fwd(st, 2 * n_edge, field->n_volumes_, VoidP(field->feat_pool_h_), I32P(field->prim_pool_),
                              I32P(field->feat_local_idx_), I32P(field->feat_local_size_), F32P(field->bias_pool_),
                              F32P(field->level_scale_), F32P(fr.pts_all), I32P(fr.vol_all), 1, VoidP(field->mlp_->params_h_),
                              F32P(feat), nullptr, VoidP(field_x)));
-    const at::Half* cache = field->prepass_x_.data_ptr<at::Half>();
     const int64_t row = (int64_t) N_LEVELS * N_CHANNELS;
     if (reuse) {
-      x_cache = field->prepass_x_;
+      x_cache = planes ? field->prepass_planes_ : field->prepass_x_;
       feat_h_cache = field->prepass_feat_h_;
       n_feat_reuse_steps_++;
       const at::Half* fh = feat_h_cache.data_ptr<at::Half>();
@@ -75,6 +75,7 @@
                              edges_ride ? static_cast<const void*>(fh + (int64_t) F2N_MLP_OUT_PAD * fr.edge_cache_row) : nullptr,
                              edges_ride ? F32P(feat) : nullptr));
     } else {
+      const at::Half* cache = field->prepass_x_.data_ptr<at::Half>();
       F2N_TIMED_CALL("field_shade_fwd", f2n_field_shade_fwd_extra(st, n_kept, n_dev, I32P(fr.src_rows),
                              static_cast<const void*>(cache + row * fr.sample_cache_row), VoidP(field->mlp_->params_h_), F32P(es.dirs),
                              fr.emb ? F32P(app) : nullptr, fr.emb ? I32P(fr.sample_emb_idx) : nullptr, VoidP(shader->mlp_->params_h_),
@@ -129,10 +130,22 @@
   F2nStepTail tail;
   const bool fused_tail = fr.dyn && step_tail_builder_ && !digest_taps_ && step_tail_builder_(&tail);
   const int64_t xrow = (int64_t) N_LEVELS * N_CHANNELS;
+  const int64_t xstep = planes ? 4 : xrow;
   const void* x_edge = !reuse || n_edge == 0 ? nullptr
-                       : edges_ride ? static_cast<const void*>(x_cache.data_ptr<at::Half>() + xrow * fr.edge_cache_row) : VoidP(field_x);
-  const void* x_surv = reuse ? static_cast<const void*>(x_cache.data_ptr<at::Half>() + xrow * fr.sample_cache_row) : nullptr;
-  if (fused_tail && reuse) {
+                       : edges_ride ? static_cast<const void*>(x_cache.data_ptr<at::Half>() + xstep * fr.edge_cache_row) : VoidP(field_x);
+  const void* x_surv = reuse ? static_cast<const void*>(x_cache.data_ptr<at::Half>() + xstep * fr.sample_cache_row) : nullptr;
+  const int plane_rows = planes ? (int) x_cache.size(1) : 0;
+  const bool edge_in_planes = planes && n_edge > 0 && edges_ride;
+  if (fused_tail && planes) {
+    field->grad_clean_ = false;
+    F2N_TIMED_CALL("field_bwd", f2n_field_bwd_step_tail_planes(st, TailStream()->stream(), n, n_dev, 2 * n_edge, field->n_volumes_, I32P(field->prim_pool_),
+                           I32P(field->feat_local_idx_), I32P(field->feat_local_size_), F32P(field->bias_pool_),
+                           F32P(field->level_scale_), F32P(fr.pts_all), I32P(fr.vol_all), 1, VoidP(field->mlp_->params_h_),
+                           edge_in_planes ? nullptr : x_edge, edge_in_planes ? x_edge : nullptr, x_surv, plane_rows, I32P(fr.src_rows),
+                           F32P(dfeat), field->mlp_->loss_scale_, F32P(field->mlp_->grad_scaled_), VoidP(field->grad_h_),
+                           field->pool_size_ / N_LEVELS, &tail, nullptr));
+    step_tail_done_ = true;
+  } else if (fused_tail && reuse) {
     field->grad_clean_ = false;
     F2N_TIMED_CALL("field_bwd", f2n_field_bwd_step_tail_rows(st, TailStream()->stream(), n, n_dev, 2 * n_edge, field->n_volumes_, I32P(field->prim_pool_),
                            I32P(field->feat_local_idx_), I32P(field->feat_local_size_), F32P(field->bias_pool_),
@@ -148,6 +161,15 @@
                            VoidP(field_x), F32P(dfeat), field->mlp_->loss_scale_, F32P(field->mlp_->grad_scaled_),
                            VoidP(field->grad_h_), field->pool_size_ / N_LEVELS, &tail, nullptr));
     step_tail_done_ = true;
+  } else if (planes) {
+    field->grad_clean_ = false;
+    F2N_TIMED_CALL("field_bwd", f2n_field_bwd_dyn_planes(st, n, n_dev, 2 * n_edge, field->n_volumes_, I32P(field->prim_pool_),
+                           I32P(field->feat_local_idx_), I32P(field->feat_local_size_), F32P(field->bias_pool_),
+                           F32P(field->level_scale_), F32P(fr.pts_all), I32P(fr.vol_all), 1, VoidP(field->mlp_->params_h_),
+                           edge_in_planes ? nullptr : x_edge, edge_in_planes ? x_edge : nullptr, x_surv, plane_rows, I32P(fr.src_rows),
+                           F32P(dfeat), field->mlp_->loss_scale_, F32P(field->mlp_->grad_scaled_), VoidP(field->grad_h_),
+                           field->pool_size_ / N_LEVELS, 1));
+    F2N_TIMED_CALL("reduce_partials", f2n_reduce_deferred(st));
   } else if (reuse) {
     field->grad_clean_ = false;
     F2N_TIMED_CALL("field_bwd", f2n_field_bwd_dyn_rows(st, n, n_dev, 2 * n_edge, field->n_volumes_, I32P(field->prim_pool_),
diff --git a/f2-nerf_amd/csrc/host/bindings.cpp b/f2-nerf_amd/csrc/host/bindings.cpp
--- a/f2-nerf_amd/csrc/host/bindings.cpp
+++ b/f2-nerf_amd/csrc/host/bindings.cpp
@@ -458,6 +458,18 @@
              Tensor none = torch::empty({0}, torch::kFloat16);
              return std::vector<Tensor>{f->prepass_x_.defined() ? f->prepass_x_ : none, f->prepass_feat_h_.defined() ? f->prepass_feat_h_ : none};
            })
+      .def("density_prepass_planes",
+           [](ExpRunner& r, const Tensor& warped, const Tensor& anchors) {
+             py::gil_scoped_release no_gil;
+             r.FinishPending();
+             return FieldOf(r)->QueryDensityPreAct(warped, anchors, true, true, true);
+           },
+           py::arg("warped"), py::arg("anchors"))
+      .def("prepass_planes",
+           [](ExpRunner& r) {
+             auto* f = FieldOf(r);
+             return f->prepass_planes_.defined() ? f->prepass_planes_ : torch::empty({0}, torch::kFloat16);
+           })
       .def("density_grid",
            [](ExpRunner& r, const std::vector<float>& lo, const std::vector<float>& hi, int res) {
              py::gil_scoped_release no_gil;
@@ -710,6 +722,9 @@
       .def_property("prepass_feat_reuse",
                     [](ExpRunner& r) { return r.renderer_->prepass_feat_reuse_; },
                     [](ExpRunner& r, bool on) { r.renderer_->prepass_feat_reuse_ = on; })
+      .def_property("prepass_planes_cache",
+                    [](ExpRunner& r) { return r.renderer_->prepass_planes_cache_; },
+                    [](ExpRunner& r, bool on) { r.renderer_->prepass_planes_cache_ = on; })
       .def_property_readonly("prepass_reuse_steps", [](ExpRunner& r) { return r.renderer_->n_feat_reuse_steps_; })
       .def_readwrite("spec_start_without_event", &ExpRunner::spec_start_without_event_)
       .def_readwrite("draws_off_main", &ExpRunner::draws_off_main_)
diff --git a/include/f2n_abi.h b/include/f2n_abi.h
--- a/include/f2n_abi.h
+++ b/include/f2n_abi.h
@@ -387,6 +387,19 @@
                                  const void* mlp_params_h, const void* x_edge_h, const void* x_cache_h, const int32_t* src_rows,
                                  const float* dfeat, float loss_scale, float* dparams_f32_scaled, void* grad_table_h, int level_entries,
                                  const F2nStepTail* tail, int* table_stepped_by_owners );
+int f2n_field_bwd_dyn_planes(void* stream, int n_max, const int32_t* n_dev, int n_off, int n_volumes, const int32_t* prim_pool,
+                             const int32_t* local_idx, const int32_t* local_size, const float* bias_pool, const float* level_scale,
+                             const float* pts_warped, const int32_t* volume_idx, int vol_stride, const void* mlp_params_h,
+                             const void* x_edge_h , const void* x_edge_planes_h , const void* x_planes_h,
+                             int plane_rows, const int32_t* src_rows, const float* dfeat, float loss_scale, float* dparams_f32_scaled,
+                             void* grad_table_h, int level_entries, int defer_reduce);
+int f2n_field_bwd_step_tail_planes(void* stream, void* tail_stream , int n_max, const int32_t* n_dev, int n_off, int n_volumes,
+                                   const int32_t* prim_pool, const int32_t* local_idx, const int32_t* local_size, const float* bias_pool,
+                                   const float* level_scale, const float* pts_warped, const int32_t* volume_idx, int vol_stride,
+                                   const void* mlp_params_h, const void* x_edge_h , const void* x_edge_planes_h ,
+                                   const void* x_planes_h, int plane_rows, const int32_t* src_rows, const float* dfeat, float loss_scale,
+                                   float* dparams_f32_scaled, void* grad_table_h, int level_entries, const F2nStepTail* tail,
+                                   int* table_stepped_by_owners );
 int f2n_adam_step_h16grad(void* stream, int n, float* param, void* grad_h, float grad_scale, float* exp_avg,
                           float* exp_avg_sq, int step, float lr, double beta1, double beta2, float eps,
                           float weight_decay, void* param_h, int zero_grad, const int32_t* skip_flag );
```

After: 705.1 million ray-samples/s (median of 6 runs). 1.01x the previous value.
